# SimonRennotte/Data-Efficient-Reinforcement-Learning-with-Probabilistic-Model-Predictive-Control

Hardware: AMD Instinct MI355X
Metric: MPC trajectory rollouts/sec (higher is better)
Workload: dtype f64

## Files before the change

### data-efficient-reinforcement-learning-with-probabilistic-model-predictive-control_amd/_lib.py

```python
import ctypes as C
import os

_HERE = os.path.dirname(os.path.abspath(__file__))
LIB_PATH = os.environ.get("GPMPC_LIB") or os.path.join(_HERE, "libgpmpc_hip.so")

GPMPC_OK = 0
GPMPC_ERR_ARG = -1
GPMPC_ERR_NOT_PD = -2
GPMPC_ERR_HIP = -3
GPMPC_ERR_LIMIT = -4


class GpmpcError(RuntimeError):
    def __init__(self, code, msg):
        super().__init__(f"gpmpc error {code}: {msg}")
        self.code = code


class NotPositiveDefiniteError(GpmpcError):
    """Cholesky failure of K + noise*I -- the reference lets torch.linalg.cholesky's error
    propagate uncaught (rl_gp_mpc/control_objects/models/gp_model.py:427)."""


_P = C.c_void_p
_D = C.c_double
_I = C.c_int

SIGNATURES = {
    "gpmpc_abi_version": (C.c_int, []),
    "gpmpc_create": (C.c_int, [C.POINTER(_P), _I]),
    "gpmpc_destroy": (C.c_int, [_P]),
    "gpmpc_last_error": (C.c_char_p, [_P]),
    "gpmpc_prepare": (C.c_int, [_P, _P, _P, _P, _P, _P, _I, _I, _I, _P]),
    "gpmpc_prepare_sparse": (C.c_int, [_P, _P, _P, _I, _P, _I, _P, _P, _P, _D, _I, _I, _P]),
    "gpmpc_sparse_append": (C.c_int, [_P, _P, _P, _I, _I, _I, _P]),
    "gpmpc_sparse_forget": (C.c_int, [_P, _P, _P, _I, _I, _I, _P]),
    "gpmpc_select_inducing": (C.c_int, [_P, _P, _I, _I, _P, _P, _D, _I, _I, _P, _P, _P, _P]),
    "gpmpc_set_factors": (C.c_int, [_P, _P, _P, _P, _P, _P, _I, _I, _I, _P]),
    "gpmpc_get_factors": (C.c_int, [_P, C.POINTER(_P), C.POINTER(_P)]),
    "gpmpc_read_factors": (C.c_int, [_P, _P, _P, _P]),
    "gpmpc_predict": (C.c_int, [_P, _P, _I, _I, _I, _P, _P, _P, _P]),
    "gpmpc_predict_backward": (C.c_int, [_P, _P, _I, _I, _I, _P, _P, _P, _P]),
    "gpmpc_predict_cov": (C.c_int, [_P, _P, _I, _P, _I, _I, _I, _P, _P, _P]),
    "gpmpc_moments": (C.c_int, [_P, _P, _P, _I, _I, _I, _P, _P, _P, _P]),
    "gpmpc_moments_linear": (C.c_int, [_P, _P, _P, _I, _I, _I, _P, _P, _P, _P]),
    "gpmpc_moments_backward": (C.c_int, [_P, _P, _P, _I, _I, _I, _P, _P, _P, _P, _P, _P]),
    "gpmpc_moments_linear_backward": (C.c_int, [_P, _P, _P, _I, _I, _I, _P, _P, _P, _P, _P, _P]),
    "gpmpc_forget": (C.c_int, [_P, C.POINTER(_I), _I, _P]),
    "gpmpc_last_prepare_mode": (C.c_int, [_P]),
    "gpmpc_last_rollout_path": (C.c_int, [_P]),
    "gpmpc_last_grad_path": (C.c_int, [_P]),
    "gpmpc_last_cluster": (C.c_int, [_P]),
    "gpmpc_build_id": (C.c_char_p, []),
    "gpmpc_mll": (C.c_int, [_P, _P, _P, _P, _P, _P, _I, _I, _I, C.POINTER(_D), _P]),
    "gpmpc_set_option": (C.c_int, [_P, C.c_char_p, C.c_longlong]),
    "gpmpc_set_cost": (C.c_int, [_P, _P, _P, _P, _D, _I, _P, _P, _I, _I]),
    "gpmpc_rollout": (C.c_int, [_P, _P, _P, _P, _I, _I, _I, _I, _D, _P, _P, _P, _P, _P, _P]),
    "gpmpc_rollout_linear": (C.c_int, [_P, _P, _P, _P, _I, _I, _I, _I, _D, _P, _P, _P, _P, _P, _P]),
    "gpmpc_rollout_linear_feedback": (C.c_int, [_P, _P, _P, _I, _P, _P, _I, _I, _I, _I, _D, _P, _P, _P, _P, _P, _P]),
    "gpmpc_lqr_gains": (C.c_int, [_P, _P, _P, _I, _I, _I, _I, _D, _D, _P, _P, _P, _P]),
    "gpmpc_rollout_grad": (C.c_int, [_P, _P, _P, _P, _I, _I, _I, _I, _D, _P, _P, _P, _P, _P, _P, _P]),
    "gpmpc_rollout_backward": (C.c_int, [_P, _P, _P, _P, _I, _I, _I, _I, _D, _P, _P, _P, _P, _P, _P, _P, _P, _P]),
    "gpmpc_rollout_linear_backward": (C.c_int, [_P, _P, _P, _P, _I, _I, _I, _I, _D, _P, _P, _P, _P, _P, _P, _P, _P, _P]),
    "gpmpc_rollout_linear_feedback_backward": (C.c_int, [_P, _P, _P, _I, _P, _P, _I, _I, _I, _I, _D, _P, _P, _P, _P, _P, _P, _P, _P,
                                                         _P, _P]),
    "gpmpc_objective_grad_host": (C.c_int, [_P, _P, _P, _P, _I, _I, _I, _D, C.POINTER(C.POINTER(_D)), _P]),
    "gpmpc_rollout_timed": (C.c_int, [_P, _P, _P, _P, _I, _I, _I, _I, _D, _P, _I, C.POINTER(C.c_float), _P]),
    "gpmpc_cem_search": (C.c_int, [_P, _P, _P, _I, _I, _I, _I, _D, _I, _I, C.c_ulonglong, _P, _I, _P, _P, _P, _P, _P]),
    "gpmpc_cem_local": (C.c_int, [_P, _P, _P, _I, _I, _I, _I, _I, _I, _D, _I, _I, C.c_ulonglong, _P, _I, _P, _P, _P, _P, _P, _P]),
    "gpmpc_cem_merge": (C.c_int, [_P, _P, _I, _I, _I, _I, _P, _P]),
    "gpmpc_argmin_async": (C.c_int, [_P, _P, _I, C.c_longlong, _P, _I, _P, _P]),
    "gpmpc_argmin_export": (C.c_int, [_P, _P, _I, C.c_longlong, _P, _I, _P, _P, _P]),
    "gpmpc_argmin": (C.c_int, [_P, _P, _I, C.c_longlong, C.POINTER(_D), C.POINTER(C.c_longlong), _P]),
}


ABI_VERSION = 24


def load(path=LIB_PATH):
    if not os.path.exists(path):
        raise ImportError(
            f"{path} not found: the HIP extension is required (no CPU fallback). "
            "Build it with `python __graft_entry__.py` or `make -C <package>/csrc`.")
    lib = C.CDLL(path)
    for name, (res, args) in SIGNATURES.items():
        fn = getattr(lib, name)
        fn.restype = res
        fn.argtypes = args
    if lib.gpmpc_abi_version() != ABI_VERSION:
        raise ImportError(f"{path}: ABI version {lib.gpmpc_abi_version()} != expected {ABI_VERSION}; rebuild the HIP library")
    return lib


_lib = None


def lib():
    global _lib
    if _lib is None:
        _lib = load()
    return _lib
```

### data-efficient-reinforcement-learning-with-probabilistic-model-predictive-control_amd/csrc/abi.hip

```cpp
#include <cmath>
#include <cstring>
#include <new>
#include <dlfcn.h>

#include "gpmpc_internal.h"
#include "lqr_gains_plan.h"

namespace {
struct Roctx {
    int (*push)(const char*) = nullptr;
    int (*pop)() = nullptr;
    Roctx() {
        for (const char* lib : {"librocprofiler-sdk-roctx.so", "libroctx64.so"}) {
            void* hnd = dlopen(lib, RTLD_LAZY | RTLD_LOCAL);
            if (!hnd) continue;
            push = reinterpret_cast<int (*)(const char*)>(dlsym(hnd, "roctxRangePushA"));
            pop = reinterpret_cast<int (*)()>(dlsym(hnd, "roctxRangePop"));
            if (push && pop) return;
            push = nullptr; pop = nullptr;
        }
    }
};
struct Range {
    static const Roctx& api() { static Roctx r; return r; }
// ... 222 lines not shown
    GPMPC_HIP_CHECK(h, hipSetDevice(h->device));
    const size_t DN = (size_t)h->D * h->N;
    if (iK_dst) GPMPC_HIP_CHECK(h, hipMemcpyAsync(iK_dst, h->iK.p, DN * h->N * sizeof(double), hipMemcpyDeviceToDevice, (hipStream_t)stream));
    if (beta_dst) GPMPC_HIP_CHECK(h, hipMemcpyAsync(beta_dst, h->beta.p, DN * sizeof(double), hipMemcpyDeviceToDevice, (hipStream_t)stream));
    return GPMPC_OK;
}

int gpmpc_predict(gpmpc_t* g, const double* Xq, int M, int D, int E, const double* noises_host, double* mean_out,
                  double* var_out, void* stream) {
    Range roctx_range("gpmpc_predict");
    if (!g) return GPMPC_ERR_ARG;
    Handle* h = H_(g);
    if (!h->ready) return bad(g, "predict before prepare / set_factors / mll");
    if (D != h->D || E != h->E) return bad(g, "predict: D / E differ from the cached model");
    if (M < 0) return bad(g, "predict: M < 0");
    if (M > 0 && !Xq) return bad(g, "null argument");
    if (M == 0) return GPMPC_OK;
    GPMPC_HIP_CHECK(h, hipSetDevice(h->device));
    return run_predict(h, Xq, M, noises_host, mean_out, var_out, (hipStream_t)stream);
}

int gpmpc_predict_backward(gpmpc_t* g, const double* Xq, int M, int D, int E, const double* mean_bar, const double* var_bar,
                           double* Xq_bar_out, void* stream) {
    Range roctx_range("gpmpc_predict_backward");
    if (!g) return GPMPC_ERR_ARG;
    Handle* h = H_(g);
    if (!h->ready) return bad(g, "predict_backward before prepare / set_factors / mll");
    if (D != h->D || E != h->E) return bad(g, "predict_backward: D / E differ from the cached model");
    if (M < 0) return bad(g, "predict_backward: M < 0");
    if (M > 0 && (!Xq || !Xq_bar_out)) return bad(g, "null argument");
    if (M == 0) return GPMPC_OK;
    GPMPC_HIP_CHECK(h, hipSetDevice(h->device));
    return run_predict_backward(h, Xq, M, mean_bar, var_bar, Xq_bar_out, (hipStream_t)stream);
}

int gpmpc_predict_cov(gpmpc_t* g, const double* Xa, int Ma, const double* Xb, int Mb, int D, int E, const double* noises_host,
                      double* cov_out, void* stream) {
    Range roctx_range("gpmpc_predict_cov");
    if (!g) return GPMPC_ERR_ARG;
    Handle* h = H_(g);
    if (!h->ready) return bad(g, "predict_cov before prepare / set_factors / mll");
    if (D != h->D || E != h->E) return bad(g, "predict_cov: D / E differ from the cached model");
    if (Ma < 0 || (Xb && Mb < 0)) return bad(g, "predict_cov: negative number of points");
    if (Xb && noises_host) return bad(g, "predict_cov: the cross form takes no noise");
    if (Ma > (1 << 22) || (Xb && Mb > (1 << 22))) return bad(g, "predict_cov: more than 2^22 points");
    if (Ma == 0 || (Xb && Mb == 0)) return GPMPC_OK;
    if (!Xa || !cov_out) return bad(g, "null argument");
    GPMPC_HIP_CHECK(h, hipSetDevice(h->device));
    return run_predict_cov(h, Xa, Ma, Xb, Mb, noises_host, cov_out, (hipStream_t)stream);
}

int gpmpc_moments(gpmpc_t* g, const double* mu, const double* var, int P, int D, int E, double* M_out, double* S_out,
                  double* V_out, void* stream) {
    Range roctx_range("gpmpc_moments");
    if (!g) return GPMPC_ERR_ARG;
    Handle* h = H_(g);
    if (!h->ready) return bad(g, "moments before prepare / set_factors / mll");
    if (D > GPMPC_MAX_D || E > GPMPC_MAX_E) {
        h->err = "moments: D or E beyond the compiled limits";
        return GPMPC_ERR_LIMIT;
    }
    if (D != h->D || E != h->E) return bad(g, "moments: D / E differ from the cached model");
    if (P < 0) return bad(g, "moments: P < 0");
    if (P > 0 && (!mu || !M_out)) return bad(g, "null argument");
    if (P == 0) return GPMPC_OK;
    GPMPC_HIP_CHECK(h, hipSetDevice(h->device));
    return run_moments(h, mu, var, P, M_out, S_out, V_out, (hipStream_t)stream);
}

int gpmpc_moments_linear(gpmpc_t* g, const double* mu, const double* var, int P, int D, int E, double* M_out, double* S_out,
                         double* V_out, void* stream) {
    Range roctx_range("gpmpc_moments_linear");
    if (!g) return GPMPC_ERR_ARG;
    Handle* h = H_(g);
    if (!h->ready) return bad(g, "moments_linear before prepare / set_factors / mll");
    if (D > GPMPC_MAX_D || E > GPMPC_MAX_E) {
        h->err = "moments_linear: D or E beyond the compiled limits";
        return GPMPC_ERR_LIMIT;
    }
    if (D != h->D || E != h->E) return bad(g, "moments_linear: D / E differ from the cached model");
    if (P < 0) return bad(g, "moments_linear: P < 0");
    if (P > 0 && !mu) return bad(g, "null argument");
    if (P == 0) return GPMPC_OK;
    GPMPC_HIP_CHECK(h, hipSetDevice(h->device));
    return run_moments_linear(h, mu, var, P, M_out, S_out, V_out, (hipStream_t)stream);
}

int gpmpc_moments_backward(gpmpc_t* g, const double* mu, const double* var, int P, int D, int E, const double* M_bar,
                           const double* S_bar, const double* V_bar, double* mu_bar_out, double* var_bar_out, void* stream) {
    Range roctx_range("gpmpc_moments_backward");
    if (!g) return GPMPC_ERR_ARG;
    Handle* h = H_(g);
    if (!h->ready) return bad(g, "moments_backward before prepare / set_factors / mll");
    if (D > GPMPC_MAX_D || E > GPMPC_MAX_E) {
        h->err = "moments_backward: D or E beyond the compiled limits";
        return GPMPC_ERR_LIMIT;
    }
    if (D != h->D || E != h->E) return bad(g, "moments_backward: D / E differ from the cached model");
    if (P < 0) return bad(g, "moments_backward: P < 0");
    if (P > 0 && !mu) return bad(g, "null argument");
    if (P == 0) return GPMPC_OK;
    GPMPC_HIP_CHECK(h, hipSetDevice(h->device));
    return run_moments_backward(h, mu, var, P, M_bar, S_bar, V_bar, mu_bar_out, var_bar_out, (hipStream_t)stream);
}

int gpmpc_moments_linear_backward(gpmpc_t* g, const double* mu, const double* var, int P, int D, int E, const double* M_bar,
                                  const double* S_bar, const double* V_bar, double* mu_bar_out, double* var_bar_out,
                                  void* stream) {
    Range roctx_range("gpmpc_moments_linear_backward");
    if (!g) return GPMPC_ERR_ARG;
    Handle* h = H_(g);
    if (!h->ready) return bad(g, "moments_linear_backward before prepare / set_factors / mll");
    if (D > GPMPC_MAX_D || E > GPMPC_MAX_E) {
        h->err = "moments_linear_backward: D or E beyond the compiled limits";
        return GPMPC_ERR_LIMIT;
    }
    if (D != h->D || E != h->E) return bad(g, "moments_linear_backward: D / E differ from the cached model");
    if (P < 0) return bad(g, "moments_linear_backward: P < 0");
    if (P > 0 && !mu) return bad(g, "null argument");
    if (P == 0) return GPMPC_OK;
    GPMPC_HIP_CHECK(h, hipSetDevice(h->device));
    return run_moments_linear_backward(h, mu, var, P, M_bar, S_bar, V_bar, mu_bar_out, var_bar_out, (hipStream_t)stream);
}

int gpmpc_mll(gpmpc_t* g, const double* X, const double* Y, const double* ls, const double* os, const double* noise,
              int N, int D, int E, double* out_host, void* stream) {
    Range roctx_range("gpmpc_mll");
    if (!g) return GPMPC_ERR_ARG;
    if (!X || !Y || !ls || !os || !noise || !out_host) return bad(g, "null argument");
    int rc = check_dims(g, N, D, E);
    if (rc) return rc;
    GPMPC_HIP_CHECK(H_(g), hipSetDevice(g->h.device));
    return run_mll(H_(g), X, Y, ls, os, noise, N, D, E, out_host, (hipStream_t)stream);
}

int gpmpc_forget(gpmpc_t* g, const int* idx_host, int k, void* stream) {
    Range roctx_range("gpmpc_forget");
    if (!g) return GPMPC_ERR_ARG;
    Handle* h = H_(g);
    if (!h->ready || !h->have_state) return bad(g, "forget: the handle holds no record of a gpmpc_prepare");
    if (!idx_host) return bad(g, "null argument");
    if (k < 1 || k >= h->N) return bad(g, "forget: need 1 <= k < N");
    for (int q = 0; q < k; ++q)
        if (idx_host[q] < 0 || idx_host[q] >= h->N || (q > 0 && idx_host[q] <= idx_host[q - 1]))
            return bad(g, "forget: indices must be strictly ascending and in [0, N)");
    GPMPC_HIP_CHECK(h, hipSetDevice(h->device));
    return run_forget(h, idx_host, k, (hipStream_t)stream);
}

int gpmpc_last_prepare_mode(gpmpc_t* g) { return g ? g->h.last_prepare_mode : GPMPC_ERR_ARG; }

int gpmpc_last_rollout_path(gpmpc_t* g) { return g ? g->h.last_rollout_path : GPMPC_ERR_ARG; }
int gpmpc_last_cluster(gpmpc_t* g) { return g ? g->h.last_cluster : GPMPC_ERR_ARG; }

int gpmpc_last_grad_path(gpmpc_t* g) { return g ? g->h.last_grad_path : GPMPC_ERR_ARG; }

#ifndef GPMPC_BUILD_ID
#define GPMPC_BUILD_ID "unknown"
#endif
const char* gpmpc_build_id(void) { return GPMPC_BUILD_ID; }

int gpmpc_set_cost(gpmpc_t* g, const double* target, const double* W, const double* W_T, double kappa,
                   int clip, const double* smin, const double* smax, int D, int A) {
    if (!g || !target || !W || !W_T) return bad(g, "null argument");
    if (D < 1 || A < 0 || D > kMaxD || D + A > kMaxE) return bad(g, "bad D / A");
    if ((smin == nullptr) != (smax == nullptr)) return bad(g, "state_min and state_max must both be given or both be NULL");
    Handle* h = H_(g);
    GPMPC_HIP_CHECK(h, hipSetDevice(h->device));
    const int DA = D + A;
    const size_t n = (size_t)DA + (size_t)DA * DA + (size_t)D * D + 2 * (size_t)D;
    int rc = grow(h, h->cost, n);
    if (rc) return rc;
    double host[kMaxE + kMaxE * kMaxE + kMaxD * kMaxD + 2 * kMaxD];
    double* q = host;
    memcpy(q, target, DA * sizeof(double)); q += DA;
    memcpy(q, W, (size_t)DA * DA * sizeof(double)); q += DA * DA;
    memcpy(q, W_T, (size_t)D * D * sizeof(double)); q += D * D;
    for (int d = 0; d < D; ++d) q[d] = smin ? smin[d] : 0.0;
    q += D;
    for (int d = 0; d < D; ++d) q[d] = smax ? smax[d] : 0.0;
    GPMPC_HIP_CHECK(h, hipMemcpy(h->cost.p, host, n * sizeof(double), hipMemcpyHostToDevice));
    h->cost_D = D; h->cost_A = A; h->kappa = kappa; h->clip = clip; h->use_constraints = smin ? 1 : 0;
    return GPMPC_OK;
}

static int fill_args(gpmpc_t* g, RolloutArgs& a, const double* actions, const double* mu0, const double* S0,
                     int B, int H, int A, int include_time, double time0, bool need_cost = true) {
    Handle* h = H_(g);
    if (!h->ready) return bad(g, "rollout before prepare / set_factors");
    if (!actions || !mu0 || !S0) return bad(g, "null argument");
    if (B < 1 || H < 1 || A < 0) return bad(g, "need B >= 1, H >= 1");
    if (h->D + A + (include_time ? 1 : 0) != h->E) return bad(g, "D + A (+1 with time) must equal the model's input dim E");
    if (need_cost && (h->cost_D != h->D || h->cost_A != A)) return bad(g, "gpmpc_set_cost not called for this (D, A)");
    memset(&a, 0, sizeof a);
    a.Xt = h->Xt.p; a.beta = h->beta.p; a.Tm = h->Tm.p; a.ils2 = h->ils2.p; a.var = h->var.p; a.logvar = h->logvar.p;
    a.cost = h->cost.p; a.kappa = h->kappa; a.clip = h->clip; a.use_constraints = h->use_constraints;
    a.actions = actions;
    a.N = h->N; a.D = h->D; a.A = A; a.E = h->E; a.H = H; a.B = B;
    a.include_time = include_time; a.time0 = time0;
    memcpy(a.mu0, mu0, h->D * sizeof(double));
    memcpy(a.S0, S0, (size_t)h->D * h->D * sizeof(double));
    return GPMPC_OK;
}

int gpmpc_rollout(gpmpc_t* g, const double* actions, const double* mu0, const double* S0, int B, int H, int A,
                  int include_time, double time0, double* mu_out, double* Sig_out, double* cm_out, double* cv_out,
                  double* J_out, void* stream) {
    Range roctx_range("gpmpc_rollout");
    if (!g) return GPMPC_ERR_ARG;
    RolloutArgs a;
    int rc = fill_args(g, a, actions, mu0, S0, B, H, A, include_time, time0, cm_out || cv_out || J_out);
    if (rc) return rc;
    GPMPC_HIP_CHECK(H_(g), hipSetDevice(g->h.device));
    a.mu_out = mu_out; a.Sig_out = Sig_out; a.cm_out = cm_out; a.cv_out = cv_out; a.J_out = J_out;
    return launch_rollout(H_(g), a, (hipStream_t)stream);
}

int gpmpc_rollout_linear(gpmpc_t* g, const double* actions, const double* mu0, const double* S0, int B, int H, int A,
                         int include_time, double time0, double* mu_out, double* Sig_out, double* cm_out, double* cv_out,
                         double* J_out, void* stream) {
    Range roctx_range("gpmpc_rollout_linear");
    if (!g) return GPMPC_ERR_ARG;
    RolloutArgs a;
    int rc = fill_args(g, a, actions, mu0, S0, B, H, A, include_time, time0, cm_out || cv_out || J_out);
    if (rc) return rc;
    GPMPC_HIP_CHECK(H_(g), hipSetDevice(g->h.device));
    a.mu_out = mu_out; a.Sig_out = Sig_out; a.cm_out = cm_out; a.cv_out = cv_out; a.J_out = J_out;
    return run_rollout_linear(H_(g), a, (hipStream_t)stream);
}

int gpmpc_rollout_linear_feedback(gpmpc_t* g, const double* actions, const double* gains, int gains_per_candidate,
                                  const double* mu0, const double* S0, int B, int H, int A, int include_time, double time0,
                                  double* mu_out, double* Sig_out, double* cm_out, double* cv_out, double* J_out, void* stream) {
    if (!gains)
        return gpmpc_rollout_linear(g, actions, mu0, S0, B, H, A, include_time, time0, mu_out, Sig_out, cm_out, cv_out, J_out,
                                    stream);
    Range roctx_range("gpmpc_rollout_linear_feedback");
    if (!g) return GPMPC_ERR_ARG;
    RolloutArgs a;
    int rc = fill_args(g, a, actions, mu0, S0, B, H, A, include_time, time0, cm_out || cv_out || J_out);
    if (rc) return rc;
    if (A < 1) return bad(g, "feedback gains need A >= 1");
    GPMPC_HIP_CHECK(H_(g), hipSetDevice(g->h.device));
    a.mu_out = mu_out; a.Sig_out = Sig_out; a.cm_out = cm_out; a.cv_out = cv_out; a.J_out = J_out;
    return run_rollout_linear(H_(g), a, (hipStream_t)stream, gains, gains_per_candidate != 0);
}

int gpmpc_lqr_gains(gpmpc_t* g, const double* actions, const double* mu0, int B, int H, int A, int include_time, double time0,
                    double reg, double* gains_out, double* P_out, int* flags_out, void* stream) {
    Range roctx_range("gpmpc_lqr_gains");
    if (!g) return GPMPC_ERR_ARG;
    Handle* h = H_(g);
    if (!h->ready) return bad(g, "lqr_gains before prepare / set_factors");
    if (!actions || !mu0 || !gains_out) return bad(g, "null argument");
    if (B < 1 || H < 1 || A < 1) return bad(g, "lqr_gains: need B >= 1, H >= 1, A >= 1");
    if (h->D + A + (include_time ? 1 : 0) != h->E) return bad(g, "D + A (+1 with time) must equal the model's input dim E");
    if (!(reg >= 0.0) || !std::isfinite(reg)) return bad(g, "lqr_gains: reg must be finite and >= 0");
    if (A > kLqrMaxA) {
        h->err = "lqr_gains: A beyond the compiled limit (A <= 8)";
        return GPMPC_ERR_LIMIT;
    }
    if (h->cost_D != h->D || h->cost_A != A) return bad(g, "gpmpc_set_cost not called for this (D, A)");
    GPMPC_HIP_CHECK(h, hipSetDevice(h->device));
    return run_lqr_gains(h, actions, mu0, B, H, A, include_time, time0, reg, gains_out, P_out, flags_out, (hipStream_t)stream);
}

int gpmpc_rollout_grad(gpmpc_t* g, const double* actions, const double* mu0, const double* S0, int B, int H, int A,
                       int include_time, double time0, double* J_out, double* grad_out, double* mu_out, double* Sig_out,
                       double* cm_out, double* cv_out, void* stream) {
    Range roctx_range("gpmpc_rollout_grad");
    if (!g) return GPMPC_ERR_ARG;
    if (!grad_out) return bad(g, "null argument");
    RolloutArgs a;
    int rc = fill_args(g, a, actions, mu0, S0, B, H, A, include_time, time0);
    if (rc) return rc;
    if (A < 1) return bad(g, "gradient needs A >= 1");
    GPMPC_HIP_CHECK(H_(g), hipSetDevice(g->h.device));
    a.mu_out = mu_out; a.Sig_out = Sig_out; a.J_out = J_out; a.cm_out = cm_out; a.cv_out = cv_out;
    return launch_rollout_grad(H_(g), a, grad_out, (hipStream_t)stream);
}

int gpmpc_rollout_backward(gpmpc_t* g, const double* actions, const double* mu0, const double* S0, int B, int H, int A,
                           int include_time, double time0, const double* mu_bar, const double* Sig_bar, const double* cm_bar,
                           const double* cv_bar, const double* J_bar, double* actions_bar_out, double* mu0_bar_out,
                           double* S0_bar_out, void* stream) {
    Range roctx_range("gpmpc_rollout_backward");
    if (!g) return GPMPC_ERR_ARG;
    if (!actions_bar_out) return bad(g, "null argument");
    RolloutSeeds sd{mu_bar, Sig_bar, cm_bar, cv_bar, J_bar, mu0_bar_out, S0_bar_out, cm_bar || cv_bar || J_bar};
    RolloutArgs a;
    int rc = fill_args(g, a, actions, mu0, S0, B, H, A, include_time, time0, sd.cost);
    if (rc) return rc;
    if (A < 1) return bad(g, "gradient needs A >= 1");
    GPMPC_HIP_CHECK(H_(g), hipSetDevice(g->h.device));
    return launch_rollout_grad(H_(g), a, actions_bar_out, (hipStream_t)stream, &sd);
}

int gpmpc_rollout_linear_backward(gpmpc_t* g, const double* actions, const double* mu0, const double* S0, int B, int H, int A,
                                  int include_time, double time0, const double* mu_bar, const double* Sig_bar,
                                  const double* cm_bar, const double* cv_bar, const double* J_bar, double* actions_bar_out,
                                  double* mu0_bar_out, double* S0_bar_out, void* stream) {
    Range roctx_range("gpmpc_rollout_linear_backward");
    if (!g) return GPMPC_ERR_ARG;
    if (!actions_bar_out) return bad(g, "null argument");
    RolloutSeeds sd{mu_bar, Sig_bar, cm_bar, cv_bar, J_bar, mu0_bar_out, S0_bar_out, cm_bar || cv_bar || J_bar};
    RolloutArgs a;
// ... 260 lines not shown
```

### data-efficient-reinforcement-learning-with-probabilistic-model-predictive-control_amd/csrc/gpmpc_internal.h

```cpp
#pragma once
#include <hip/hip_runtime.h>
#include <cstddef>
#include <cstdio>
#include <string>
#include <unordered_set>

#include "../../include/gpmpc.h"

namespace gpmpc_hip {

constexpr int kMaxD = GPMPC_MAX_D;
constexpr int kMaxE = GPMPC_MAX_E;
constexpr int kWave = 64;

struct ClusterMap {
    int CS, D, P, P_off, wpp, wtri, koff;
    int CSd;
    unsigned char sepown[8];
    unsigned char meanown[4];
    unsigned char dmem[32];
    unsigned char didx[32];
    __host__ __device__ int diag_owner(int ord, int slot) const { return dmem[((ord * wtri + slot) * CSd) / (D * wtri)]; }
    __host__ __device__ int off_owner(int ord, int slot) const { return ((slot * koff) / wpp + ord * koff) % CS; }
    __host__ __device__ int sep_owner(int ord) const { return sepown[ord]; }
// ... 33 lines not shown
                for (int k = 1; k < koff; ++k) {
                    const int m = (o * koff + k) % CS;
                    if (diag_count(m) <= diag_count(best)) best = m;
                }
            sepown[o] = (unsigned char)best;
            taken[best] = true;
        }
        if (dedicated) {
            CSd = 0;
            for (int m = 0; m < 32; ++m) didx[m] = 255;
            for (int m = 0; m < CS; ++m)
                if (!taken[m]) { dmem[CSd] = (unsigned char)m; didx[m] = (unsigned char)CSd; ++CSd; }
        }
        for (int a = 0; a < D && a < 4; ++a) {
            int pick = -1;
            for (int m = CS - 1, k = 0; m >= 0 && pick < 0; --m)
                if (!taken[m]) { if (k == a) pick = m; ++k; }
            meanown[a] = (unsigned char)(pick >= 0 ? pick : (a * CS / D) % CS);
        }
    }
};

constexpr int kInlineActs = 64;
struct RolloutArgs {
    const double* Xt;
    const double* beta;
    const double* Tm;
    const double* ils2;
    const double* var;
    const double* logvar;
    const double* cost;
    double kappa;
    int clip;
    int use_constraints;
    const double* actions;
    int N, D, A, E, H, B;
    int B_plan;
    int include_time;
    double time0;
    double* mu_out;
    double* Sig_out;
    double* cm_out;
    double* cv_out;
    double* J_out;
    const double* xrange;
    const int* mono_exp;
    const double* mono_w;
    int mono_cum[16];
    int sep_kmax;
    int CM;
    int force_path;
    int force_sep;
    int x_in_lds;
    int cols2;
    int G;
    int CH;
    int RC;
    unsigned magic_N;
    unsigned magic_wpp;
    unsigned magic_pt;
    int tiled;
    int t_begin, t_end;
    int ntiles;
    const double* tile_part;
    const int* slow;
    double* grad_mom;
    int* grad_done;
    int grad_NSP, grad_NXP;
    int cluster;
    ClusterMap cmap;
    int cl_slots;
    int xch_n;
    unsigned xch_tag0;
    unsigned long long* xch;
    unsigned long long* xch_uc;
    int cl_dbg;
    int act_inline_n;
    double* act_store;
    double act_inline[kInlineActs];
    double mu0[kMaxD];
    double S0[kMaxD * kMaxD];
};

struct Buf {
    double* p = nullptr;
    size_t cap = 0;
};

struct Handle {
    int device = 0;
    std::string err;
    int N = 0, D = 0, E = 0;
    bool ready = false;
    Buf Xt;
    Buf beta;
    Buf iK;
    Buf Tm;
    Buf ils2;
    Buf var;
    Buf logvar;
    Buf gram;
    Buf linv;
    Buf zvec;
    Buf cost;
    Buf best;
    Buf traj;
    Buf xrange;
    Buf gradws;
    Buf mllws;
    Buf cemws;
    Buf tilews;
    Buf tgradws;
    Buf predws;
    Buf predbws;
    Buf covws;
    Buf momws;
    Buf mombws;
    Buf linws;
    Buf linbws;
    Buf lqrws;
    struct SepTable* septab = nullptr;
    Buf sepw;
    int septab_D = -1, sep_ks = 0, sep_cmax = 0;
    hipStream_t side_stream = nullptr;
    hipEvent_t ev_params = nullptr, ev_points = nullptr;
    Buf Xc, Yc;
    Buf hyp;
    Buf kv, vv;
    Buf sc;
    int* mismatch = nullptr;
    int inc_updates = 0;
    bool have_state = false;
    Buf Xf, Yf;
    Buf fgws;
    Buf spws;
    Buf selws;
    int* fidx = nullptr;
    size_t fidx_cap = 0;
    Buf hio;
    double* hio_host = nullptr;
    double* hio_host_dev = nullptr;
    size_t hio_host_cap = 0;
    unsigned long long* hio_flag = nullptr;
    unsigned long long* hio_flag_dev = nullptr;
    unsigned long long hio_seq = 0;
    double* hx_out = nullptr; const double* hx_src = nullptr; int hx_n = 0;
    Buf xch;
    unsigned long long* xch_uc = nullptr;
    size_t xch_uc_cap = 0;
    unsigned xch_epoch = 1;
    int opt_cluster = 0;
    int opt_cl_dbg = 0;
    int last_cluster = 1;
    Buf mono_w;
    int* mono_exp = nullptr;
    int mono_D = -1;
    int mono_cum[16] = {0};
    int sep_kmax = 0;
    int mono_CM = 0;
    int* info = nullptr;
    std::unordered_set<const void*> lds_configured;
    int cost_D = -1, cost_A = -1;
    double kappa = 1.0;
    int clip = 0;
    int use_constraints = 0;
    int opt_threads = 0;
    int opt_lds_kb = 0;
    int opt_force_global = 0;
    int opt_rows_per_chunk = 0;
    int opt_force_path = 0;
    int opt_force_sep = 0;
    int opt_grad_stream = 0;
    int opt_grad_share = 0;
    int opt_grad_chunk = 0;
    int chunk_key[8] = {0, 0, 0, 0, 0, 0, 0, 0};
    int chunk_rows = 0;
    int opt_grad_tiles = 1;
    int opt_grad_sep = 1;
    int opt_cols_per_lane = 0;
    int opt_incremental = 1;
    int opt_refresh_every = 32;
    int opt_outer2 = 2;
    int opt_outer_min_n = 640;
    int opt_block128 = 1;
    int opt_inner_left = 1;
    int opt_tile128 = 1;
    int opt_outer_block = 1;
    int opt_pair_tiles = 0;
    int last_rollout_path = 0;
    int opt_grad_mean = 1;
    int last_grad_path = 0;
    int opt_prepare_inv_batch = 4;
    int opt_prepare_invcols = 1;
    int opt_prepare_fuse = 1;
    int opt_prepare_overlap = 1;
    int opt_gram_shared = 1;
    int opt_fused_prepare = 1;
    int last_prepare_mode = 0;
    int opt_sparse_chunk = 0;
    long long opt_select_max_mb = 0;
    int opt_predict_chunk = 0;
    int opt_predict_bwd_chunk = 0;
    int opt_predict_cov_chunk = 0;
    int opt_moments_chunk = 0;
    int opt_moments_bwd_chunk = 0;
    int opt_moments_linear_chunk = 0;
    int opt_moments_linear_bwd_chunk = 0;
    int opt_lqr_gains_chunk = 0;
    int lds_limit = 160 * 1024;
    int num_cu = 256;
    Buf sprec;
    bool sp_have = false;
    size_t sp_yu = 0;
    Buf spupd;
};

inline int allow_full_lds(Handle* h, const void* kernel);

#define GPMPC_HIP_CHECK(h, expr)                                                         \
    do {                                                                                 \
        hipError_t e_ = (expr);                                                          \
        if (e_ != hipSuccess) {                                                          \
            (h)->err = std::string(#expr) + ": " + hipGetErrorString(e_);                \
            return GPMPC_ERR_HIP;                                                        \
        }                                                                                \
    } while (0)

inline int allow_full_lds(Handle* h, const void* kernel) {
    if (h->lds_configured.count(kernel)) return GPMPC_OK;
    GPMPC_HIP_CHECK(h, hipFuncSetAttribute(kernel, hipFuncAttributeMaxDynamicSharedMemorySize, h->lds_limit));
    h->lds_configured.insert(kernel);
    return GPMPC_OK;
}

inline unsigned magic_div(unsigned d) { return d <= 1 ? 0u : (unsigned)((0x100000000ULL + d - 1) / d); }

constexpr double kTileTableBytes = 6.0e6;
inline bool tables_outgrow_l2(int N, int D) { return 4.0 * D * (double)N * N >= kTileTableBytes; }

struct RolloutRequest {
    bool fused_tiles;
    bool costs_to_caller;
};
struct RolloutPlan {
    int DP;
    int nt;
    int path;
    int cols2, G, CH, RC, x_in_lds;
    size_t lds_bytes;
    int cluster, cl_slots, xch_n;
    ClusterMap cmap;
    unsigned magic_N, magic_wpp, magic_pt;
    int CM, sep_kmax;
    bool fused_tiles;
    bool costs_to_caller;
    const char* err;
};

struct MomTiling {
    int G, CH, RC, wpp, gz;
    size_t lds;
};
struct GradPlan {
    int DP, NXP, RS, NSP;
    int sweep_nt, pre_steps;
    size_t sweep_lds;
    bool stream;
    size_t gs_lds;
    MomTiling first;
    MomTiling pass;
    bool share_cu;
    bool tiles, fused;
    bool sep;
    int sep_kmax, sep_NA, sep_NE, sep_PS, sep_wave_words;
    size_t sep_lds;
    int pairs_left;
    bool few, merged;
    int path;
    RolloutPlan fwd;
};

constexpr int kSmallPathMaxN = 240;
constexpr int kSmallCholeskyMinN = 96;
constexpr int kInvColsMaxN = 352;
constexpr int kInvColsWideMaxN = 544;
constexpr int kSyrkTiledMinN = 512;
constexpr int kGramSharedTilesPerCu = 2;

enum class PreparePath {
    small_whole,
    small_cholesky,
    panel32,
    outer,
};
enum class GramForm { full, lower, shared_lower };
enum class Inv32Form { rows, cols, side };
enum class OuterInvForm { rows128, doubling, doubling_ykk };
enum class SyrkInvForm { w32, tiled, t128 };
struct PreparePlan {
    PreparePath path;
    GramForm gram;
    bool round2;
    bool fuse_next;
    Inv32Form inv32;
    int inv_batch;
    bool tile128;
// ... 101 lines not shown
```

### data-efficient-reinforcement-learning-with-probabilistic-model-predictive-control_amd/csrc/rollout.hip

```cpp
#include "rollout_stream_kernel.h"

namespace gpmpc_hip {

int launch_rollout_dp2(Handle*, RolloutArgs&, int, bool, size_t, hipStream_t);
int launch_rollout_dp3(Handle*, RolloutArgs&, int, bool, size_t, hipStream_t);
int launch_rollout_dp4(Handle*, RolloutArgs&, int, bool, size_t, hipStream_t);
int launch_rollout_dp6(Handle*, RolloutArgs&, int, bool, size_t, hipStream_t);
int launch_rollout_dp8(Handle*, RolloutArgs&, int, bool, size_t, hipStream_t);
int launch_rollout_dp16(Handle*, RolloutArgs&, int, bool, size_t, hipStream_t);

__global__ __launch_bounds__(64) void traj_cost_kernel(const double* __restrict__ mu, const double* __restrict__ Sig,
                                                       const double* __restrict__ actions, const double* __restrict__ cost,
                                                       int D, int A, int H, double kappa, int clip, int use_constraints,
                                                       double* __restrict__ cm_out, double* __restrict__ cv_out,
                                                       double* __restrict__ J_out) {
    traj_cost_body(blockIdx.x, threadIdx.x, mu, Sig, actions, cost, D, A, H, kappa, clip, use_constraints, cm_out, cv_out, J_out);
}

__device__ __forceinline__ void keep_better(double& bv, long long& bi, double ov, long long oi) {
    if (oi >= 0 && (bi < 0 || ov < bv || (ov == bv && oi < bi))) { bv = ov; bi = oi; }
}

__global__ __launch_bounds__(1024) void argmin_kernel(const double* J, int B, long long first, double* out, int index_as_double,
                                                     const double* actions, int HA, double* out_host) {
// ... 231 lines not shown
        const int items = D * wtri, P_off = D * (D - 1) / 2;
        const int cs_floor = (P_off + 2 * D > 9) ? P_off + 2 * D : 9;
        const bool roomy = cap >= cs_floor;
        int cs = 1;
        if (h.opt_cluster >= 2) cs = h.opt_cluster;
        else if (items >= 24 || (roomy && items * D >= 18)) {
            cs = (items + 3) / 4;
            if (roomy && cs < cs_floor) cs = cs_floor;
        }
        if (cs > 32) cs = 32;
        if (cs > cap) cs = cap;
        for (const int cs_min = h.opt_cluster >= 2 ? cs : (cs + 1) / 2; cs >= 2 && cs >= cs_min && cluster == 1; --cs) {
            p.cmap.plan(cs, D, wpp_c, wtri);
            p.cl_slots = 0;
            for (int m = 0; m < cs; ++m) { const int n = p.cmap.slots_needed(m); if (n > p.cl_slots) p.cl_slots = n; }
            for (int xl = ((size_t)E * N * 8 <= 32 * 1024) ? 1 : 0; xl >= 0 && cluster == 1; --xl) {
                const Layout L = make_layout(N, D, A, E, P, DP, wpp_c, CM, CH, H * A, xl != 0, true, p.cl_slots);
                if ((size_t)L.lds_total * 8 <= lds_cap) { G = P; lds_bytes = (size_t)L.lds_total * 8; p.x_in_lds = xl; cluster = cs; }
            }
        }
        if (cluster > 1 && h.opt_threads == 0) nt = cluster >= 8 ? 512 : 1024;
        if (cluster == 1) cl_chunks = false;
    }
    if (!gs && cluster == 1) {
        choose_layout(false);
        if (G == 0) { gs = true; tiled = false; }
    }
    if (gs) {
        if (DP % 4 == 0 && DP >= 8) {
            CH = (N >= 1024) ? 256 : 64;
            if (h.opt_rows_per_chunk > 0) CH = h.opt_rows_per_chunk <= 64 ? 64 : (h.opt_rows_per_chunk <= 128 ? 128 : 256);
        } else {
            CH = (N >= 64) ? 64 : ((N + 3) & ~3);
        }
        RC = (N + CH - 1) / CH;
        G = 1;
        StreamLayout SL = make_stream_layout(N, D, A, E, DP, CH, H * A);
        lds_bytes = (size_t)SL.total * 8;
        if (lds_bytes > (size_t)h.lds_limit) { p.err = "rollout: N too large for the LDS column-factor array"; return GPMPC_ERR_LIMIT; }
        nt = 1024;
    }
    p.cols2 = (cols2 && !gs) ? 1 : 0;
    const int NCf = p.cols2 ? NCu : N;
    const unsigned wppv = (unsigned)((RC * NCf + 63) / 64);
    p.magic_N = magic_div((unsigned)NCf);
    p.magic_wpp = magic_div(wppv);
    p.magic_pt = magic_div((unsigned)N);
    if ((unsigned long long)RC * NCf * NCf >= 0x100000000ULL || (unsigned long long)G * wppv * wppv >= 0x100000000ULL ||
        (!gs && (unsigned long long)(D + 2 * P) * N * N >= 0x100000000ULL)) {
        p.err = "rollout: index range too large for the multiply-high division"; return GPMPC_ERR_LIMIT;
    }
    if (!gs && (unsigned long long)G * wppv >= 65000ULL) {
        p.err = "rollout: too many work-item slots for the 16-bit item list"; return GPMPC_ERR_LIMIT;
    }
    p.nt = nt; p.path = gs ? 1 : (tiled ? 2 : 0);
    p.G = G; p.CH = CH; p.RC = RC; p.lds_bytes = lds_bytes;
    p.cluster = cluster;
    if (cluster > 1) p.xch_n = G * (int)wppv + G + D * (D + 1) + 32;
    p.fused_tiles = tiled && req.fused_tiles;
    p.costs_to_caller = req.costs_to_caller;
    return GPMPC_OK;
}

static int exchange_buffers(Handle* h, RolloutArgs& a, const RolloutPlan& p, hipStream_t s) {
    const size_t words = (size_t)8 * ((a.B + 7) / 8) * 4 * p.xch_n;
    const bool fresh = !h->xch.p || words > h->xch.cap;
    int rc = grow(h, h->xch, words);
    if (rc) return rc;
    const bool wrap = h->xch_epoch >= (1u << 19) - 1;
    if (fresh || wrap) { rc = zero_exchange(h, reinterpret_cast<unsigned long long*>(h->xch.p), h->xch.cap, s); if (rc) return rc; }
    if (words > h->xch_uc_cap) {
        if (h->xch_uc) GPMPC_HIP_CHECK(h, hipFree(h->xch_uc));
        h->xch_uc = nullptr; h->xch_uc_cap = 0;
        void* q = nullptr;
        if (hipExtMallocWithFlags(&q, words * sizeof(unsigned long long), hipDeviceMallocUncached) != hipSuccess) {
            (void)hipGetLastError();
            GPMPC_HIP_CHECK(h, hipExtMallocWithFlags(&q, words * sizeof(unsigned long long), hipDeviceMallocFinegrained));
        }
        h->xch_uc = reinterpret_cast<unsigned long long*>(q);
        h->xch_uc_cap = words;
        rc = zero_exchange(h, h->xch_uc, words, s);
        if (rc) return rc;
    } else if (wrap) {
        rc = zero_exchange(h, h->xch_uc, h->xch_uc_cap, s);
        if (rc) return rc;
    }
    if (wrap) h->xch_epoch = 1;
    a.xch_tag0 = h->xch_epoch * 8192u;
    h->xch_epoch += 1;
    a.xch = reinterpret_cast<unsigned long long*>(h->xch.p);
    a.xch_uc = h->xch_uc;
    return GPMPC_OK;
}

int launch_rollout(Handle* h, RolloutArgs& a, const RolloutPlan& p, hipStream_t s) {
    const bool tiled = p.path == 2;
    a.xrange = h->xrange.p; a.mono_exp = h->mono_exp; a.mono_w = h->mono_w.p;
    for (int k = 0; k < 16; ++k) a.mono_cum[k] = h->mono_cum[k];
    a.sep_kmax = p.sep_kmax; a.CM = p.CM;
    a.force_path = h->opt_force_path; a.force_sep = h->opt_force_sep;
    a.x_in_lds = p.x_in_lds; a.cols2 = p.cols2;
    a.G = p.G; a.CH = p.CH; a.RC = p.RC;
    a.magic_N = p.magic_N; a.magic_wpp = p.magic_wpp; a.magic_pt = p.magic_pt;
    a.cluster = p.cluster; a.cmap = p.cmap; a.cl_slots = p.cl_slots; a.cl_dbg = h->opt_cl_dbg;
    a.xch = nullptr; a.xch_uc = nullptr; a.xch_n = p.xch_n; a.xch_tag0 = 0;
    a.tiled = tiled ? 1 : 0;
    if (!p.fused_tiles) a.grad_mom = nullptr;
    if (!tiled) { a.t_begin = 0; a.t_end = 0; a.slow = nullptr; a.tile_part = nullptr; a.ntiles = 0; }
    if (a.act_inline_n > 0 && p.path != 0) {
        InlineActs u;
        for (int i = 0; i < kInlineActs; ++i) u.v[i] = a.act_inline[i];
        hipLaunchKernelGGL(inline_acts_kernel, dim3(1), dim3(64), 0, s, a.act_store, a.act_inline_n, u);
        GPMPC_HIP_CHECK(h, hipGetLastError());
        a.act_inline_n = 0;
    }
    if (!a.mu_out || !a.Sig_out) {
        const size_t nmu = (size_t)a.B * (a.H + 1) * a.D, nS = nmu * a.D;
        int rc = grow(h, h->traj, nmu + nS);
        if (rc) return rc;
        if (!a.mu_out) a.mu_out = h->traj.p;
        if (!a.Sig_out) a.Sig_out = h->traj.p + nmu;
    }
    int rc = p.cluster > 1 ? exchange_buffers(h, a, p, s) : GPMPC_OK;
    if (rc) return rc;
    auto launch_kernel = [&]() {
        const bool gs = p.path == 1;
        switch (p.DP) {
            case 2:  return launch_rollout_dp2(h, a, p.nt, gs, p.lds_bytes, s);
            case 3:  return launch_rollout_dp3(h, a, p.nt, gs, p.lds_bytes, s);
            case 4:  return launch_rollout_dp4(h, a, p.nt, gs, p.lds_bytes, s);
            case 6:  return launch_rollout_dp6(h, a, p.nt, gs, p.lds_bytes, s);
            case 8:  return launch_rollout_dp8(h, a, p.nt, gs, p.lds_bytes, s);
            default: return launch_rollout_dp16(h, a, p.nt, gs, p.lds_bytes, s);
        }
    };
    if (tiled) {
        rc = tile_workspace(h, a);
        if (!rc) rc = launch_tile_state_init(h, a, s);
        for (int t = 0; t < a.H && !rc; ++t) {
            rc = launch_pair_tiles(h, a, t, s);
            a.t_begin = t; a.t_end = t + 1;
            if (!rc) rc = launch_kernel();
        }
    } else {
        rc = launch_kernel();
    }
    if (rc) return rc;
    if ((a.cm_out || a.cv_out || a.J_out) && !p.costs_to_caller) {
        rc = launch_traj_cost(h, a, a.cm_out, a.cv_out, a.J_out, s);
        if (rc) return rc;
    }
    h->last_rollout_path = p.path;
    h->last_cluster = p.cluster;
    return GPMPC_OK;
}

int launch_rollout(Handle* h, RolloutArgs& a, hipStream_t s) {
    int rc = ensure_rollout_tables(h, a.N, a.D);
    if (rc) return rc;
    RolloutPlan p;
    rc = plan_rollout(*h, a.N, a.D, a.A, a.E, a.H, a.B_plan > a.B ? a.B_plan : a.B, RolloutRequest{false, false}, p);
    if (rc) { h->err = p.err; return rc; }
    return launch_rollout(h, a, p, s);
}

}
```

### data-efficient-reinforcement-learning-with-probabilistic-model-predictive-control_amd/csrc/rollout_kernel.h

```cpp
#pragma once
#include "device_common.h"

#if defined(GPMPC_PROF_ON)
#define GPMPC_TRACE(id) do { if (threadIdx.x == 0 && blockIdx.x == 0) { long long now_ = __builtin_readcyclecounter(); \
    prof_acc[id] += now_ - prof_last; prof_last = now_; } \
    if (CL && threadIdx.x == 0 && (blockIdx.x & 7) == 0) { long long w_ = wall_clock64(); prof_wall[id] += w_ - prof_wlast; prof_wlast = w_; } } while (0)
#else
#define GPMPC_TRACE(id) do {} while (0)
#endif

namespace gpmpc_hip {

typedef const __attribute__((address_space(3))) double* lds_cptr;
__device__ inline double lds_b64(const double* p) {
    lds_cptr q = (lds_cptr)p;
    asm volatile("" : "+v"(q));
    return *q;
}

typedef double lds_d2 __attribute__((ext_vector_type(2)));
template <int NL, int NV>
__device__ inline void lds_load_pairs(const double* rec, double (&v)[NV]) {
    static_assert(NV >= ((NL + 1) & ~1), "destination too short");
    const lds_d2* r2 = reinterpret_cast<const lds_d2*>(rec);
// ... 435 lines not shown
#pragma unroll
        for (int u = 0; u < U; ++u) {
            double r[RS];
            REC::template load<RS>(rec + u * RS, r);
            double x = r[REC::EA] + kb0, y = r[REC::EA] + kb1;
#pragma unroll
            for (int d = 0; d < DP; ++d) { x = fma(r[REC::G + d], w0[d], x); y = fma(r[REC::G + d], w1[d], y); }
            a0[u] = x; a1[u] = y;
            if (diag) t_row_pair(t, so + (unsigned)u * t.row_bytes, wt0[u], wt1[u]);
            else { wt0[u] = r[REC::RA]; wt1[u] = r[REC::RA]; }
        }
#pragma unroll
        for (int u = 0; u < U; ++u) {
            acc0 = fma(fast_exp(a0[u], tab), wt0[u], acc0);
            acc1 = fma(fast_exp(a1[u], tab), wt1[u], acc1);
        }
        rec += U * RS;
        so += (unsigned)U * t.row_bytes;
    }
}

__device__ inline double wave_sum8(const double (&v)[8], int lane) {
    auto xchg = [](double x, int mask) { return __shfl_xor(x, mask, 64); };
    const bool b0 = lane & 1, b1 = lane & 2, b2 = lane & 4;
    double r4[4], r2[2];
#pragma unroll
    for (int k = 0; k < 4; ++k) {
        const double keep = b0 ? v[k + 4] : v[k], send = b0 ? v[k] : v[k + 4];
        r4[k] = keep + xchg(send, 1);
    }
#pragma unroll
    for (int k = 0; k < 2; ++k) {
        const double keep = b1 ? r4[k + 2] : r4[k], send = b1 ? r4[k] : r4[k + 2];
        r2[k] = keep + xchg(send, 2);
    }
    double r = (b2 ? r2[1] : r2[0]) + xchg(b2 ? r2[0] : r2[1], 4);
    r += xchg(r, 8);
    r += xchg(r, 16);
    r += xchg(r, 32);
    return r;
}

constexpr int sep3_bands(int KS) { return KS <= 3 ? 2 : (KS == 4 ? 3 : (KS == 5 ? 5 : 7)); }
constexpr int sep3_i0(int B, int KS) {
    if (KS <= 4) return B;
    if (KS == 5) return B < 2 ? 0 : B - 1;
    return B < 2 ? 0 : (B < 4 ? 1 : B - 2);
}
constexpr int sep3_i1(int B, int KS) { return B == sep3_bands(KS) - 1 ? KS : sep3_i0(B, KS); }
constexpr int sep3_j0(int B, int KS) {
    if (KS == 5) return B == 1 ? 2 : 0;
    if (KS >= 6) return (B == 1 || B == 3) ? 2 : 0;
    return 0;
}
constexpr int sep3_j1(int B, int KS) {
    if (KS == 5) return B == 0 ? 1 : KS;
    if (KS >= 6) return (B == 0 || B == 2) ? 1 : KS;
    return KS;
}
constexpr int sep3_count(int B, int KS) {
    int n = 0;
    if (B >= sep3_bands(KS)) return 0;
    for (int i = sep3_i0(B, KS); i <= sep3_i1(B, KS) && i <= KS; ++i)
        for (int j = sep3_j0(B, KS); j <= sep3_j1(B, KS) && j <= KS - i; ++j) n += KS - i - j + 1;
    return n;
}
template <int KS, int B>
struct Sep3Canon {
    int v[sep3_count(B, KS) > 0 ? sep3_count(B, KS) : 1];
    constexpr Sep3Canon() : v{} {
        int n = 0;
        for (int i = sep3_i0(B, KS); i <= sep3_i1(B, KS) && i <= KS && B < sep3_bands(KS); ++i)
            for (int j = sep3_j0(B, KS); j <= sep3_j1(B, KS) && j <= KS - i; ++j)
                for (int kk = 0; kk <= KS - i - j; ++kk) {
                    const int deg = i + j + kk;
                    const int cum = deg * (deg + 1) * (deg + 2) / 6;
                    v[n++] = cum + (deg - i) * (deg - i + 1) / 2 + (deg - i - j);
                }
    }
};

template <int KS, int B>
__device__ inline void sep3_band(int lane, int N, int side, const double* rec0, int RS, const double* kb, const double* nu,
                                 const double* il, double* mom) {
    constexpr int NBm = sep3_count(B, KS);
    if constexpr (NBm > 0) {
        constexpr int NP = (NBm + 7) & ~7;
        constexpr int I0 = sep3_i0(B, KS), I1 = sep3_i1(B, KS) < KS ? sep3_i1(B, KS) : KS;
        constexpr int J0 = sep3_j0(B, KS), J1 = sep3_j1(B, KS);
        double acc[NP];
#pragma unroll
        for (int m = 0; m < NP; ++m) acc[m] = 0.0;
        for (int pt = lane; pt < N; pt += 64) {
            double x0, x1, x2, wt;
            if (side == 0) {
                double r[RowRecAligned<3>::RS];
                RowRecAligned<3>::load<RowRecAligned<3>::RS>(rec0 + (size_t)pt * RS, r);
                wt = r[RowRecAligned<3>::RA]; x0 = r[0]; x1 = r[1]; x2 = r[2];
            } else {
                wt = kb[pt];
                x0 = nu[pt] * il[0]; x1 = nu[N + pt] * il[1]; x2 = nu[2 * N + pt] * il[2];
            }
            double py[KS + 1], pz[KS + 1];
            py[0] = 1.0; pz[0] = 1.0;
#pragma unroll
            for (int e = 1; e <= KS; ++e) { py[e] = py[e - 1] * x1; pz[e] = pz[e - 1] * x2; }
            double wx = wt;
#pragma unroll
            for (int e = 0; e < I0; ++e) wx *= x0;
            int n = 0;
#pragma unroll
            for (int i = I0; i <= I1; ++i) {
#pragma unroll
                for (int j = J0; j <= (J1 < KS - i ? J1 : KS - i); ++j) {
                    const double aij = wx * py[j];
#pragma unroll
                    for (int kk = 0; kk <= KS - i - j; ++kk) { acc[n] = fma(aij, pz[kk], acc[n]); ++n; }
                }
                wx *= x0;
            }
        }
        static constexpr Sep3Canon<KS, B> canon{};
        const int mq = lane >> 2;
#pragma unroll
        for (int g16 = 0; g16 + 16 <= NP; g16 += 16) {
            const double(&grp)[16] = *reinterpret_cast<const double(*)[16]>(&acc[g16]);
            const double tot = wave_reduce16(grp);
            if ((lane & 3) == 0 && g16 + mq < NBm) mom[canon.v[g16 + mq]] = tot;
        }
        if constexpr (NP % 16 != 0) {
            constexpr int g8 = NP - 8;
            const double(&grp)[8] = *reinterpret_cast<const double(*)[8]>(&acc[g8]);
            const double tot = wave_reduce8(grp);
            if ((lane & 3) == 0 && lane < 32 && g8 + mq < NBm) mom[canon.v[g8 + mq]] = tot;
        }
    }
}

template <int KS>
__device__ __attribute__((noinline)) void sep3_item(int band, int lane, int N, int side, const double* rec0, int RS,
                                                     const double* kb, const double* nu, const double* il, double* mom) {
    switch (band) {
        case 0: sep3_band<KS, 0>(lane, N, side, rec0, RS, kb, nu, il, mom); break;
        case 1: sep3_band<KS, 1>(lane, N, side, rec0, RS, kb, nu, il, mom); break;
        case 2: sep3_band<KS, 2>(lane, N, side, rec0, RS, kb, nu, il, mom); break;
        case 3: sep3_band<KS, 3>(lane, N, side, rec0, RS, kb, nu, il, mom); break;
        case 4: sep3_band<KS, 4>(lane, N, side, rec0, RS, kb, nu, il, mom); break;
        case 5: sep3_band<KS, 5>(lane, N, side, rec0, RS, kb, nu, il, mom); break;
        default: sep3_band<KS, 6>(lane, N, side, rec0, RS, kb, nu, il, mom); break;
    }
}

template <int DP, bool CL>
constexpr int rollout_min_waves() { return (DP == 2 || (DP == 3 && !CL)) ? 4 : 1; }

template <int DP, int NT, int DX, bool C2, bool TILED = false, bool CL = false>
__global__ __launch_bounds__(NT, (rollout_min_waves<DP, CL>())) void rollout_kernel(const RolloutArgs p) {
    static_assert(!TILED || (DP <= 4 && NT >= 256), "the batch-major path is built for D <= 4");
    static_assert(!CL || (!TILED && DP <= 4 && NT >= 256), "the cooperative form is built for D <= 4");
    extern __shared__ __attribute__((aligned(16))) double smem[];
    if constexpr (TILED) {
        if (p.slow[blockIdx.x] != p.t_begin + 1) return;
    }
    constexpr int NW = NT / kWave;
    using REC = RowRecAligned<DP>;
    constexpr int RS = REC::RS;
    const int tid = threadIdx.x;
    const int CS = CL ? p.cluster : 1;
    const bool spread = CL && (p.cl_dbg & 8);
    const int member = CL ? (spread ? (int)blockIdx.x % CS : (int)(blockIdx.x >> 3) % CS) : 0;
    const int c = CL ? (spread ? (int)blockIdx.x / CS : (int)(blockIdx.x & 7) + 8 * ((int)(blockIdx.x >> 3) / CS)) : (int)blockIdx.x;
    if constexpr (CL) { if (c >= p.B) return; }
    const int D = (DX > 0) ? DX : p.D;
    const int N = p.N, A = p.A, E = p.E, H = p.H, G = p.G, CM = p.CM;
    const int P = TILED ? D * (D - 1) / 2 : D * (D + 1) / 2;
    const int DA = D + A;
    const int LD = 2 * D;
    const int NC = C2 ? (N + 1) / 2 : N;
    const int wpp = (p.RC * NC + 63) / 64;
    const int SD2 = rnd2(D * D);

    const Layout L = make_layout(N, D, A, E, G, DP, wpp, CM, p.CH, H * A, p.x_in_lds != 0, CL, CL ? p.cl_slots : 0);
    const int NR = N + p.CH;
    double* s_mu = smem + L.mu;
    double* s_Sig2 = smem + L.Sig;
    double* s_m = smem + L.m;
    double* s_M = smem + L.M;
    double* s_cc = smem + L.cc;
    double* s_s1 = smem + L.s1;
    double* s_Vs = smem + L.Vs;
    double* s_Sp = smem + L.Sp;
    double* s_rdet = smem + L.rdet;
    [[maybe_unused]] double* s_rdiag = smem + L.misc;
    double* s_aug = smem + L.aug;
    double* s_part = smem + L.part;
    double* s_mom = smem + L.mom;
    int* s_pa = reinterpret_cast<int*>(smem + L.ints);
    int* s_pb = s_pa + P;
    int* s_K = s_pb + P;
    int* s_counter = s_K + G;
    int* s_noff = s_counter + 1;
    int* s_off = s_noff + 1;
    int* s_mcum = s_off + G;
    int* s_tri = s_mcum + 16;
    int* s_nslot = s_tri + tri_ints(N);
    int* s_nitems = s_nslot + G;
    unsigned short* s_items = reinterpret_cast<unsigned short*>(
        smem + L.ints + rnd2((2 * P + 3 * G + 8 + 16 + tri_ints(N) + 1) / 2));

    [[maybe_unused]] double* s_sepv = smem + L.cl;
    [[maybe_unused]] int* s_ord = reinterpret_cast<int*>(smem + L.cl + rnd2(G));
    [[maybe_unused]] int* s_fail = reinterpret_cast<int*>(smem + L.cl + rnd2(G) + rnd2((G + 1) / 2));
    [[maybe_unused]] unsigned char* s_needw = reinterpret_cast<unsigned char*>(smem + L.cl + rnd2(G) + rnd2((G + 1) / 2) + 2);
    [[maybe_unused]] unsigned char* s_own = s_needw + kClusterScratch * 8;
    [[maybe_unused]] unsigned char* s_sepown = s_own + G * wpp;
    [[maybe_unused]] unsigned char* s_elneed = s_sepown + G;
    [[maybe_unused]] unsigned char* s_meanown = s_elneed + G;
    [[maybe_unused]] unsigned short* s_mine = reinterpret_cast<unsigned short*>(
        smem + L.cl + rnd2(G) + rnd2((G + 1) / 2) + 2 + kClusterScratch + rnd2((G * wpp + 2 * G + 16 + 7) / 8));
    [[maybe_unused]] int* s_slot = reinterpret_cast<int*>(smem + L.cl + rnd2(G) + rnd2((G + 1) / 2) + 2 + kClusterScratch +
                                                          rnd2((G * wpp + 2 * G + 16 + 7) / 8) + rnd2((G * wpp + 16 + 4 + 3) / 4));
    [[maybe_unused]] unsigned long long* s_mymask = reinterpret_cast<unsigned long long*>(
        smem + L.cl + rnd2(G) + rnd2((G + 1) / 2) + 2 + kClusterScratch + rnd2((G * wpp + 2 * G + 16 + 7) / 8) +
        rnd2((G * wpp + 16 + 4 + 3) / 4) + rnd2((G + 1) / 2));
    const int GL = CL ? p.cl_slots : G;

    [[maybe_unused]] unsigned long long* xbuf_uc = CL ? p.xch_uc + (size_t)c * 4 * p.xch_n : nullptr;
    [[maybe_unused]] unsigned long long* xbuf = CL ? p.xch + (size_t)c * 4 * p.xch_n : nullptr;
    [[maybe_unused]] const int x_sep = G * wpp, x_mean = G * wpp + G;
    [[maybe_unused]] const int x_xcc = x_mean + D * (D + 1);
    [[maybe_unused]] int* s_lmap = reinterpret_cast<int*>(smem + L.lmap);
    constexpr int LMS = CL ? kLaneMapSlotsCluster : kLaneMapSlots;
    [[maybe_unused]] int* s_lrows = s_lmap + (wpp < LMS ? wpp : LMS) * 64;
    double* ppbase = smem;
    double* a_nu = ppbase + L.nu;
    double* a_lb = ppbase + L.lb;
    double* a_rows = ppbase + L.rows;
    double* a_kb = ppbase + L.kb;

    double* c_ils2 = smem + L.c_ils2;
    double* c_logvar = smem + L.c_logvar;
    double* c_var = smem + L.c_var;
    double* c_xr = smem + L.c_xr;
    double* c_act = smem + L.c_act;
    double* c_exptab = smem + L.c_exptab;
    const double* Xs = p.x_in_lds ? (smem + L.c_X) : p.Xt;
    double* c_monow = smem + L.c_monow;
    int* c_monoe = reinterpret_cast<int*>(smem + L.c_monoe);
    const double* act = p.actions + (size_t)c * H * A;

#if defined(GPMPC_PROF_ON)
    long long prof_x[3] = {0, 0, 0};
    long long prof_acc[10] = {0, 0, 0, 0, 0, 0, 0, 0, 0, 0};
    long long prof_last = __builtin_readcyclecounter();
    long long prof_wall[10] = {0, 0, 0, 0, 0, 0, 0, 0, 0, 0};
    long long prof_wlast = wall_clock64();
#endif
    if constexpr (TILED) {
        for (int i = tid; i < D; i += NT) { s_mu[i] = p.mu_out[((size_t)c * (H + 1) + p.t_begin) * D + i]; c_logvar[i] = p.logvar[i]; c_var[i] = p.var[i]; }
        for (int i = tid; i < D * D; i += NT) s_Sig2[i] = p.Sig_out[((size_t)c * (H + 1) + p.t_begin) * D * D + i];
    }
    {
        const bool inl = p.act_inline_n > 0;
        const int CMc = CM > 0 ? CM : 0;
        const double* mw = CMc > 0 ? p.mono_w : p.ils2;
        const int* me = CMc > 0 ? p.mono_exp : reinterpret_cast<const int*>(p.ils2);
        const int im = tid < CMc ? tid : 0;
        const int nX = p.x_in_lds ? E * N : 0;
        __builtin_amdgcn_sched_barrier(0);
        const double v_lv = p.logvar[tid < D ? tid : 0], v_var = p.var[tid < D ? tid : 0];
        const double v_ils = p.ils2[tid < D * E ? tid : 0], v_xr = p.xrange[tid < 2 * E ? tid : 0];
        const double v_act = act[tid < H * A ? tid : 0];
        const double v_exp = kExp2Tab[tid & 63];
        const double v_mw = mw[im];
        const int e0 = me[im * 4], e1 = me[im * 4 + 1], e2 = me[im * 4 + 2], e3 = me[im * 4 + 3];
        const double v_x0 = p.Xt[tid < nX ? tid : 0], v_x1 = p.Xt[tid + NT < nX ? tid + NT : 0];
        [[maybe_unused]] const double v_mu0 = p.mu0[tid < D ? tid : 0], v_S0 = p.S0[tid < D * D ? tid : 0];
        __builtin_amdgcn_sched_barrier(0);
        if constexpr (!TILED) {
            if (tid < D) s_mu[tid] = v_mu0;
            if (tid < D * D) s_Sig2[tid] = v_S0;
        }
        if (tid < D) { c_logvar[tid] = v_lv; c_var[tid] = v_var; }
        if (tid < D * E) c_ils2[tid] = v_ils;
        if (tid < 2 * E) c_xr[tid] = v_xr;
        if (tid < 64) c_exptab[tid] = v_exp;
        if (tid < CMc) { c_monow[tid] = v_mw; c_monoe[tid] = e0 | (e1 << 8) | (e2 << 16) | (e3 << 24); }
        if (tid < nX) smem[L.c_X + tid] = v_x0;
        if (tid + NT < nX) smem[L.c_X + tid + NT] = v_x1;
        if (inl) {
            for (int i = tid; i < H * A; i += NT) {
                const double v = p.act_inline[i < kInlineActs ? i : 0];
                c_act[i] = v;
                if (!CL || member == 0) p.act_store[i] = v;
            }
        } else {
            if (tid < H * A) c_act[tid] = v_act;
            for (int i = tid + NT; i < H * A; i += NT) c_act[i] = act[i];
        }
        for (int i = tid + NT; i < D; i += NT) { c_logvar[i] = p.logvar[i]; c_var[i] = p.var[i]; }
        for (int i = tid + NT; i < D * E; i += NT) c_ils2[i] = p.ils2[i];
        for (int i = tid + NT; i < 2 * E; i += NT) c_xr[i] = p.xrange[i];
        for (int i = tid + 2 * NT; i < nX; i += NT) smem[L.c_X + i] = p.Xt[i];
        for (int i = tid + NT; i < CMc; i += NT) {
            c_monow[i] = p.mono_w[i];
            c_monoe[i] = p.mono_exp[i * 4] | (p.mono_exp[i * 4 + 1] << 8) | (p.mono_exp[i * 4 + 2] << 16) | (p.mono_exp[i * 4 + 3] << 24);
        }
    }
    for (int i = tid; i < GL * p.CH * RS; i += NT) {
        const int gq = i / (p.CH * RS), k = i - gq * (p.CH * RS);
        a_rows[((size_t)gq * NR + N) * RS + k] = 0.0;
    }
    if (tid >= 64 && tid < 80) s_mcum[tid - 64] = p.mono_cum[tid - 64];
    if (tid == 0) {
        int q = 0;
        [[maybe_unused]] int nd_ = 0, no_ = 0;
        for (int a = 0; a < D; ++a)
            for (int b = TILED ? a + 1 : a; b < D; ++b) {
                s_pa[q] = a; s_pb[q] = b;
                if constexpr (CL) s_ord[q] = (a == b) ? nd_++ : no_++;
                ++q;
            }
        if constexpr (CL) *s_fail = 0;
        int run = 0;
        for (int r = 0; r <= p.RC; ++r) {
            s_tri[r] = run;
            const int first = C2 ? (r * p.CH) / 2 : r * p.CH;
            run += (first < NC) ? NC - first : 0;
        }
    }
    __syncthreads();
    bool use_lmap = false;
    if constexpr (!TILED) {
        const int wtri = (s_tri[p.RC] + 63) >> 6;
        use_lmap = wtri <= LMS && wtri <= wpp;
        if (use_lmap) {
            for (int slot = tid >> 6; slot < wtri; slot += NW) {
                const int flat = slot * 64 + (tid & 63);
                const bool valid = flat < s_tri[p.RC];
                int lo = 0, hi = p.RC;
                while (hi - lo > 1) {
                    const int mid = (lo + hi) >> 1;
                    if (s_tri[mid] <= flat) lo = mid; else hi = mid;
                }
                const int r = valid ? lo : 0;
                const int first = C2 ? (r * p.CH) / 2 : r * p.CH;
                const int jc = valid ? first + (flat - s_tri[r]) : 0;
                const int j = C2 ? 2 * jc : jc;
                const int jl = (C2 && (j + 1 < N)) ? j + 1 : j;
                const int i0 = r * p.CH;
                int i1 = i0 + p.CH;
                if (i1 > N) i1 = N;
                if (i1 > jl + 1) i1 = jl + 1;
                const int len = (valid && i1 > i0) ? (i1 - i0) : 0;
                const int nrows = (wave_max_i32(len) + 3) & ~3;
                s_lmap[flat] = valid ? (r | (jc << 8)) : -1;
                if ((tid & 63) == 0) s_lrows[slot] = nrows;
            }
        }
        __syncthreads();
    }
    GPMPC_TRACE(1);
    if (!TILED && member == 0) {
        for (int i = tid; i < D; i += NT) p.mu_out[((size_t)c * (H + 1)) * D + i] = s_mu[i];
        for (int i = tid; i < D * D; i += NT) p.Sig_out[((size_t)c * (H + 1)) * D * D + i] = s_Sig2[i];
    }

    [[maybe_unused]] const int wtri_c = CL ? (s_tri[p.RC] + 63) >> 6 : 0;
    if constexpr (CL) {
        const ClusterMap& cmap = p.cmap;
        for (int i = tid; i < P * wpp; i += NT) {
            const int gq = i / wpp, slot = i - gq * wpp, ord = s_ord[gq];
            int o;
            if (s_pa[gq] == s_pb[gq]) o = slot < wtri_c ? cmap.diag_owner(ord, slot) : 255;
            else o = cmap.off_owner(ord, slot);
            s_own[i] = (unsigned char)o;
        }
        for (int gq = tid; gq < P; gq += NT) {
            const int ord = s_ord[gq];
            const bool dg = s_pa[gq] == s_pb[gq];
            s_sepown[gq] = (unsigned char)(dg ? 255 : cmap.sep_owner(ord));
            s_elneed[gq] = (dg ? cmap.diag_needed(ord, member) : cmap.off_needed(ord, member)) ? 1 : 0;
        }
        for (int a = tid; a < D; a += NT) s_meanown[a] = (unsigned char)cmap.mean_owner(a);
        __syncthreads();
        if (tid == 0) {
            int n = 0;
            for (int gq = 0; gq < P; ++gq) s_slot[gq] = s_elneed[gq] ? n++ : -1;
            if (n > GL) *s_fail = 1;
        }
        for (int gq = tid >> 6; gq < P; gq += NT / 64) {
            const int k = tid & 63;
            const int lim = (s_pa[gq] == s_pb[gq]) ? wtri_c : wpp;
            const unsigned long long m = __ballot(k < lim && k < wpp && s_own[gq * wpp + (k < wpp ? k : 0)] == member);
            if (k == 0) s_mymask[gq] = m;
        }
        __syncthreads();
    }
    [[maybe_unused]] auto item_owner = [&](int code) -> int {
        if (code >= 0xffff - 15) return s_meanown[0xffff - code];
        const int gq = p.magic_wpp ? (int)__umulhi((unsigned)code, p.magic_wpp) : code;
        return (s_K[gq] & 64) ? s_sepown[gq] : s_own[code];
    };
    [[maybe_unused]] auto pair_needed = [&](int gq) -> bool { return (s_K[gq] & 64) ? s_sepown[gq] == member : s_elneed[gq] != 0; };
    [[maybe_unused]] unsigned x_tag = 0;
    [[maybe_unused]] unsigned long long* x_cur = xbuf;
    [[maybe_unused]] bool same_xcd = false;
    [[maybe_unused]] auto publish = [&](int vi, double v) {
        unsigned long long* g = x_cur + 2 * (size_t)vi;
        const unsigned long long hi_tag = (unsigned long long)x_tag << 32;
        if (same_xcd) {
            __hip_atomic_store(g, hi_tag | (unsigned)__double2loint(v), __ATOMIC_RELAXED, __HIP_MEMORY_SCOPE_WORKGROUP);
            __hip_atomic_store(g + 1, hi_tag | (unsigned)__double2hiint(v), __ATOMIC_RELAXED, __HIP_MEMORY_SCOPE_WORKGROUP);
        } else {
            __hip_atomic_store(g, hi_tag | (unsigned)__double2loint(v), __ATOMIC_RELAXED, __HIP_MEMORY_SCOPE_AGENT);
            __hip_atomic_store(g + 1, hi_tag | (unsigned)__double2hiint(v), __ATOMIC_RELAXED, __HIP_MEMORY_SCOPE_AGENT);
        }
    };
    [[maybe_unused]] auto acquire = [&](int vi) -> double {
        const unsigned long long* g = x_cur + 2 * (size_t)vi;
        for (int spins = 0; spins < (1 << 21); ++spins) {
            const unsigned long long a = __hip_atomic_load(g, __ATOMIC_RELAXED, __HIP_MEMORY_SCOPE_AGENT);
            const unsigned long long b = __hip_atomic_load(g + 1, __ATOMIC_RELAXED, __HIP_MEMORY_SCOPE_AGENT);
            if ((unsigned)(a >> 32) == x_tag && (unsigned)(b >> 32) == x_tag) return __hiloint2double((int)(unsigned)b, (int)(unsigned)a);
            __builtin_amdgcn_s_sleep(1);
        }
        *s_fail = 1;
        return __builtin_nan("");
    };

    if constexpr (CL) {
        x_tag = p.xch_tag0;
        x_cur = xbuf + (size_t)2 * p.xch_n;
        const int my_xcc = __builtin_amdgcn_s_getreg(20 | (0 << 6) | ((4 - 1) << 11));
        if (tid == 0) publish(x_xcc + member, (double)my_xcc);
        if (tid < 64) {
            const bool differs = tid < CS && acquire(x_xcc + tid) != (double)my_xcc;
            const unsigned long long any_differs = __ballot(differs);
            if (tid == 0) s_fail[1] = (any_differs == 0 && !(p.cl_dbg & 4)) ? 1 : 0;
        }
        __syncthreads();
        same_xcd = s_fail[1] != 0;
        if (*s_fail) {
            if (member == 0) {
                for (int i = tid; i < H * D; i += NT) p.mu_out[((size_t)c * (H + 1) + 1) * D + i] = __builtin_nan("");
                for (int i = tid; i < H * D * D; i += NT) p.Sig_out[((size_t)c * (H + 1) + 1) * D * D + i] = __builtin_nan("");
            }
            return;
        }
    }

    int cur = 0;
    const int tid_outer = tid;
    for (int t = TILED ? p.t_begin : 0; t < (TILED ? p.t_end : H); ++t) {
        int tid_opaque = tid_outer;
        asm volatile("" : "+v"(tid_opaque));
        const int tid = tid_opaque;
        const int lane = tid & 63;
        const int wave = tid >> 6;
        const double* s_Sig = s_Sig2 + cur * SD2;
        double* s_SigNext = s_Sig2 + (cur ^ 1) * SD2;
        if constexpr (CL) {
            x_tag = p.xch_tag0 + (unsigned)t + 1u;
            x_cur = (same_xcd ? xbuf : xbuf_uc) + (size_t)(t & 1) * 2 * p.xch_n;
        }

        for (int q0 = 0; q0 < P || (TILED && q0 == 0); q0 += G) {
            const int Gc = (P - q0 < G) ? (P - q0) : G;
            const bool first = (q0 == 0);
            const int nmean = first ? D : 0;

            constexpr int kPairBase = (NT >= 256) ? 64 : 0;
#if defined(GPMPC_PROF_ON)
            const long long prof_p1 = __builtin_readcyclecounter();
#endif
            if (first) {
                for (int i = tid; i < E; i += NT) {
                    double v;
                    if (i < D) v = s_mu[i];
                    else if (i < DA) v = c_act[t * A + (i - D)];
                    else v = p.time0 + (double)t;
                    s_m[i] = v;
                }
            }
            if (tid < nmean) {
                const int a = tid;
                double* aug = s_aug + a * (D * LD);
                double prodil = 1.0;
                double detA;
                if constexpr (DP <= 4) {
                    double m[DP][2 * DP];
#pragma unroll
                    for (int i = 0; i < DP; ++i) {
                        const double il2 = (i < D) ? c_ils2[a * E + i] : 1.0;
                        prodil *= il2;
#pragma unroll
                        for (int j = 0; j < DP; ++j) {
                            const bool in = (i < D && j < D);
                            m[i][j] = (in ? s_Sig[i * D + j] : 0.0) + (i == j ? 1.0 / il2 : 0.0);
                            m[i][DP + j] = (in && i == j) ? 1.0 : 0.0;
                        }
                    }
                    detA = small_solve<DP>(m);
#pragma unroll
                    for (int i = 0; i < DP; ++i)
#pragma unroll
                        for (int j = 0; j < DP; ++j)
                            if (i < D && j < D) aug[i * LD + D + j] = m[i][DP + j];
                } else {
                    for (int i = 0; i < D; ++i) {
                        const double il2 = c_ils2[a * E + i];
                        prodil *= il2;
                        for (int j = 0; j < D; ++j) {
                            aug[i * LD + j] = s_Sig[i * D + j] + (i == j ? 1.0 / il2 : 0.0);
                            aug[i * LD + D + j] = (i == j ? 1.0 : 0.0);
                        }
                    }
                    detA = gauss_solve(aug, D, D, LD);
                }
                s_cc[a] = c_var[a] / sqrt(detA * prodil);
            } else if (tid >= kPairBase + (kPairBase ? 0 : nmean) && tid < kPairBase + (kPairBase ? 0 : nmean) + Gc) {
                const int gq = tid - kPairBase - (kPairBase ? 0 : nmean);
                const int a = s_pa[q0 + gq], b = s_pb[q0 + gq];
                double* aug = s_aug + (D + gq) * (D * LD);
                double detR;
                double cmax = 0.0;
                if constexpr (DP <= 4) {
                    double m[DP][2 * DP];
#pragma unroll
                    for (int i = 0; i < DP; ++i)
#pragma unroll
                        for (int j = 0; j < DP; ++j) {
                            const bool in = (i < D && j < D);
                            const double sg = in ? s_Sig[i * D + j] : 0.0;
                            const double dab = in ? c_ils2[a * E + j] + c_ils2[b * E + j] : 0.0;
                            m[i][j] = sg * dab + (i == j ? 1.0 : 0.0);
                            m[i][DP + j] = sg;
                        }
                    double ur[DP], wr[DP];
#pragma unroll
                    for (int i = 0; i < DP; ++i) {
                        const double mi = (i < D) ? s_mu[i] : 0.0;
                        const double rg = (i < D) ? fmax(fabs(c_xr[i] - mi), fabs(c_xr[E + i] - mi)) : 0.0;
                        ur[i] = (i < D) ? rg * c_ils2[a * E + i] : 0.0;
                        wr[i] = (i < D) ? rg * c_ils2[b * E + i] : 0.0;
                    }
                    detR = small_solve<DP>(m);
                    double rowc[DP];
#pragma unroll
                    for (int i = 0; i < DP; ++i) {
                        double r = 0.0;
#pragma unroll
                        for (int j = 0; j < DP; ++j) {
                            if (i < D && j < D) {
                                aug[i * LD + D + j] = m[i][DP + j];
                                r = fma(fabs(m[i][DP + j]), wr[j], r);
                            }
                        }
                        rowc[i] = r * ur[i];
                    }
#pragma unroll
                    for (int i = 0; i < DP; ++i) cmax += rowc[i];
                } else {
                    for (int i = 0; i < D; ++i)
                        for (int j = 0; j < D; ++j) {
                            const double dab = c_ils2[a * E + j] + c_ils2[b * E + j];
                            aug[i * LD + j] = s_Sig[i * D + j] * dab + (i == j ? 1.0 : 0.0);
                            aug[i * LD + D + j] = s_Sig[i * D + j];
                        }
                    detR = gauss_solve(aug, D, D, LD);
                    const double* Z = aug + D;
                    for (int i = 0; i < D; ++i) {
                        const double mi = s_mu[i];
                        const double ui = fmax(fabs(c_xr[i] - mi), fabs(c_xr[E + i] - mi)) * c_ils2[a * E + i];
                        for (int j = 0; j < D; ++j) {
                            const double mj = s_mu[j];
                            const double wj = fmax(fabs(c_xr[j] - mj), fabs(c_xr[E + j] - mj)) * c_ils2[b * E + j];
                            cmax = fma(fabs(Z[i * LD + j]) * ui, wj, cmax);
                        }
                    }
                }
                s_rdet[gq] = 1.0 / sqrt(detR);
                int K = 0;
                if (p.force_path != 1 && cmax <= kTaylorMaxArg[kMaxTaylor]) {
                    K = 1;
#pragma unroll
                    for (int k = 1; k < kMaxTaylor; ++k) K += (cmax > kTaylorMaxArg[k]) ? 1 : 0;
                }
                if (a != b && K > 0 && K <= p.sep_kmax && (DX != 3 || K <= 6) && p.force_path == 0) {
                    const long long C_ = s_mcum[K < 3 ? 3 : K];
                    const long long NBk = (s_mcum[K] + 7) / 8;
                    const long long cost_sep = (DX == 3) ? 2 * (((N + 63) / 64) * (2 * C_ + 40) + (C_ / 8 + 4) * 70)
                                                         : 2 * NBk * (((N + 63) / 64) * (6 + 8 * K) + 80);
                    const long long cost_el = (long long)N * N * (D + K + 3) / 64;
                    if (p.force_sep || cost_sep < cost_el) K |= 64;
                }
                if constexpr (CL) K |= (s_slot[gq] + 1) << 8;
                s_K[gq] = K;
            }
            if constexpr (TILED) {
                if (first && tid >= 128 && tid < 128 + D) {
                    const int a = tid - 128;
                    double m[DP][2 * DP];
#pragma unroll
                    for (int i = 0; i < DP; ++i)
#pragma unroll
                        for (int j = 0; j < DP; ++j) {
                            const bool in = (i < D && j < D);
                            const double sg = in ? s_Sig[i * D + j] : 0.0;
                            const double dab = in ? c_ils2[a * E + j] + c_ils2[a * E + j] : 0.0;
                            m[i][j] = sg * dab + (i == j ? 1.0 : 0.0);
                            m[i][DP + j] = sg;
                        }
                    s_rdiag[a] = 1.0 / sqrt(small_solve<DP>(m));
                } else if (first && wave == 3) {
                    for (int a = 0; a < D; ++a) {
                        const double* tp = p.tile_part + ((size_t)c * D + a) * p.ntiles;
                        double v = 0.0;
                        for (int k = lane; k < p.ntiles; k += 64) v += tp[k];
                        v = wave_sum(v);
                        if (lane == 0) s_rdiag[4 + a] = v;
                    }
                }
            }
#if defined(GPMPC_PROF_ON)
            if (threadIdx.x == 0 && blockIdx.x == 0) { long long now_ = __builtin_readcyclecounter(); prof_acc[7] += now_ - prof_last; }
            if (blockIdx.x == 0 && threadIdx.x == 64) prof_x[0] += __builtin_readcyclecounter() - prof_p1;
#endif
            if (tid == NT - 1) {
                *s_counter = 0;
                int no = 0;
                for (int gq = 0; gq < Gc; ++gq)
                    if (s_pa[q0 + gq] != s_pb[q0 + gq]) s_off[no++] = gq;
                *s_noff = no;
#if defined(GPMPC_PROF_ON)
                if (blockIdx.x == 0) prof_x[1] += __builtin_readcyclecounter() - prof_p1;
#endif
            }
            __syncthreads();
            GPMPC_TRACE(2);

            const int n_off = *s_noff;
            [[maybe_unused]] bool cl_list_pending = false;
            [[maybe_unused]] int cl_ns = 0, cl_cls = 3, cl_code0 = 0;
            if (wave == NW - 1) {
                const int wtri = (s_tri[p.RC] + 63) >> 6;
                const int R = Gc + nmean;
                int ns = 0, cls = 3, code0 = 0;
                [[maybe_unused]] unsigned long long mymask = 0;
                if (lane < Gc) {
                    const int Kr = s_K[lane];
                    const bool sep = (Kr & 64) != 0;
                    if (sep) {
                        const int Ks = Kr & 63;
                        const int two = (DX == 3) ? 2 * sep3_bands(Ks <= 3 ? 3 : Ks) : 2 * ((s_mcum[Ks] + 7) >> 3);
                        ns = two < wpp ? two : wpp;
                    } else {
                        ns = (s_pa[q0 + lane] == s_pb[q0 + lane]) ? wtri : wpp;
                    }
                    cls = sep ? 1 : 0;
                    code0 = lane * wpp;
                    s_nslot[lane] = ns;
                    if constexpr (CL) {
                        if (sep) mymask = (s_sepown[lane] == member) ? (ns >= 64 ? ~0ull : (1ull << ns) - 1ull) : 0ull;
                        else mymask = s_mymask[lane];
                    }
                } else if (lane < R) {
                    ns = 1; cls = 2; code0 = 0xffff - (lane - Gc);
                    if constexpr (CL) mymask = (s_meanown[lane - Gc] == member) ? 1ull : 0ull;
                }
                auto build_list = [&] {
                    int start = 0, total_items = 0;
                    for (int m = 0; m < R; ++m) {
                        const int nsm = __builtin_amdgcn_readlane(ns, m);
                        const int clm = __builtin_amdgcn_readlane(cls, m);
                        start += (clm < cls || (clm == cls && m < lane)) ? nsm : 0;
                        total_items += nsm;
                    }
                    for (int k = 0; k < ns; ++k) s_items[start + k] = (unsigned short)(cls == 2 ? code0 : code0 + k);
                    if (lane == 0) *s_nitems = total_items;
                    return total_items;
                };
                if constexpr (!CL) {
                    (void)build_list();
                } else if (wpp > 64) {
                    const int total_items = build_list();
                    wave_lds_sync();
                    int cnt = 0;
                    for (int base = 0; base < total_items; base += 64) {
                        const int k = base + lane;
                        const int code = s_items[k < total_items ? k : 0];
                        const bool mine = k < total_items && item_owner(code) == member;
                        const unsigned long long mask = __ballot(mine);
                        if (mine) s_mine[1 + cnt + __popcll(mask & ((1ull << lane) - 1ull))] = (unsigned short)code;
                        cnt += __popcll(mask);
                    }
                    if (lane == 0) s_mine[0] = (unsigned short)cnt;
                } else {
                    const int mycnt = __popcll(mymask);
                    int pre = 0, tot = 0, total_items = 0;
                    for (int m = 0; m < R; ++m) {
                        const int cm = __builtin_amdgcn_readlane(mycnt, m);
                        const int clm = __builtin_amdgcn_readlane(cls, m);
                        pre += (clm < cls || (clm == cls && m < lane)) ? cm : 0;
                        tot += cm;
                        total_items += __builtin_amdgcn_readlane(ns, m);
                    }
                    unsigned long long mk = mymask;
                    for (int i = 0; mk != 0; ++i) {
                        const int k = __builtin_ctzll(mk);
                        mk &= mk - 1ull;
                        s_mine[1 + pre + i] = (unsigned short)(cls == 2 ? code0 : code0 + k);
                    }
                    if (lane == 0) { s_mine[0] = (unsigned short)tot; *s_nitems = total_items; }
                    cl_list_pending = true;
                    cl_ns = ns; cl_cls = cls; cl_code0 = code0;
                }
            }
            const int p2_threads = (NW >= 8) ? NT - 64 : NT;
            int p2_items = (nmean + Gc + n_off) * N;
            [[maybe_unused]] bool cl_nu_first = false;
            if (CL && (NW < 8 || wave != NW - 1)) {
                const int nall = nmean + Gc + n_off;
                bool need = false;
                int code = lane;
                if (lane < nmean) need = s_meanown[lane] == member;
                else if (lane < nmean + Gc) need = pair_needed(lane - nmean);
                else if (lane < nall) need = pair_needed(s_off[lane - nmean - Gc]);
                const unsigned long long mask0 = __ballot(need);
                if (lane == nall) { need = s_meanown[0] != member && mask0 == 0; code = 255; }
                const unsigned long long mask = __ballot(need);
                if (need) s_needw[wave * 64 + __popcll(mask & ((1ull << lane) - 1ull))] = (unsigned char)code;
                p2_items = __popcll(mask) * N;
                cl_nu_first = s_meanown[0] != member && mask0 != 0;
                wave_lds_sync();
            }
            for (int it = tid; it < p2_items && tid < p2_threads; it += p2_threads) {
                int prob = p.magic_pt ? (int)__umulhi((unsigned)it, p.magic_pt) : it;
                const int pt = it - prob * N;
                double nu[DP];
#pragma unroll
                for (int d = 0; d < DP; ++d) nu[d] = (d < D) ? (Xs[d * N + pt] - s_m[d]) : 0.0;
                if constexpr (CL) {
                    if (cl_nu_first && prob == 0) {
#pragma unroll
                        for (int d = 0; d < DP; ++d)
                            if (d < D) a_nu[d * N + pt] = nu[d];
                    }
                    prob = s_needw[wave * 64 + prob];
                    if (prob == 255) {
#pragma unroll
                        for (int d = 0; d < DP; ++d)
                            if (d < D) a_nu[d * N + pt] = nu[d];
                        continue;
                    }
                }
                if (prob < nmean) {
                    const int a = prob;
                    const double* Ai = s_aug + a * (D * LD) + D;
                    double q = 0.0;
#pragma unroll
                    for (int i = 0; i < DP; ++i) {
                        if (i < D) {
                            double r = 0.0;
#pragma unroll
                            for (int j = 0; j < DP; ++j)
                                if (j < D) r = fma(Ai[i * LD + j], nu[j], r);
                            q = fma(nu[i], r, q);
                        }
                    }
                    for (int e = D; e < E; ++e) {
                        const double v = Xs[e * N + pt] - s_m[e];
                        q = fma(v * v, c_ils2[a * E + e], q);
                    }
                    a_lb[a * N + pt] = fast_exp(-0.5 * q, c_exptab) * p.beta[a * N + pt];
                    if (a == 0) {
#pragma unroll
                        for (int d = 0; d < DP; ++d)
                            if (d < D) a_nu[d * N + pt] = nu[d];
                    }
                } else {
                    const bool rowside = prob < nmean + Gc;
                    const int gq = rowside ? prob - nmean : s_off[prob - nmean - Gc];
                    const int a = s_pa[q0 + gq], b = s_pb[q0 + gq];
                    const int c = rowside ? a : b;
                    const int Kw = s_K[gq];
                    const int K = Kw & 63;
                    const int sl = CL ? (Kw >> 8) - 1 : gq;
                    const double* Z = s_aug + (D + gq) * (D * LD) + D;
                    double u[DP], g[DP];
// ... 151 lines not shown
                            } else {
                                wt = a_kb[sl3 * N + pt];
#pragma unroll
                                for (int d = 0; d < DP; ++d) x[d] = (d < D) ? a_nu[d * N + pt] * c_ils2[b * E + d] : 0.0;
                            }
#pragma unroll
                            for (int m = 0; m < 8; ++m) {
                                double t = wt;
#pragma unroll
                                for (int d = 0; d < (DP < 4 ? DP : 4); ++d) {
                                    const int ne = (packed[m] >> (8 * d)) & 255;
                                    for (int e = 0; e < ne; ++e) t *= x[d];
                                }
                                acc[m] += t;
                            }
                        }
                        const double tot = wave_reduce8(acc);
                        const int mm = lane >> 2;
                        if ((lane & 3) == 0 && lane < 32 && al0 + mm < C) s_mom[(gq * 2 + side) * rnd2(CM) + al0 + mm] = tot;
                    }
                    continue;
                }
                const int flat = slot * 64 + lane;
                bool valid;
                int r, jc;
                int nrows_tab = -1;
                if (diag && use_lmap) {
                    const int packed = s_lmap[flat];
                    valid = packed >= 0;
                    r = valid ? (packed & 255) : 0;
                    jc = valid ? (packed >> 8) : 0;
                    nrows_tab = __builtin_amdgcn_readfirstlane(s_lrows[slot]);
                } else if (diag) {
                    valid = flat < s_tri[p.RC];
                    int lo = 0, hi = p.RC;
                    while (hi - lo > 1) {
                        const int mid = (lo + hi) >> 1;
                        if (s_tri[mid] <= flat) lo = mid; else hi = mid;
                    }
                    r = valid ? lo : 0;
                    const int first = C2 ? (r * p.CH) / 2 : r * p.CH;
                    jc = valid ? first + (flat - s_tri[r]) : 0;
                } else {
                    valid = flat < p.RC * NC;
                    r = valid ? (p.magic_N ? (int)__umulhi((unsigned)flat, p.magic_N) : flat) : 0;
                    jc = valid ? flat - r * NC : 0;
                }
                const int j = C2 ? 2 * jc : jc;
                const bool valid1 = C2 && (j + 1 < N);
                const int jl = valid1 ? j + 1 : j;
                const int i0 = r * p.CH;
                int i1 = i0 + p.CH;
                if (i1 > N) i1 = N;
                if (diag && i1 > jl + 1) i1 = jl + 1;
                int nrows = nrows_tab;
                if (nrows_tab < 0) {
                    const int len = (valid && i1 > i0) ? (i1 - i0) : 0;
                    nrows = (wave_max_i32(len) + 3) & ~3;
                }
                double acc = 0.0;
                if (nrows > 0) {
                    double w[DP];
#pragma unroll
                    for (int d = 0; d < DP; ++d) w[d] = (d < D) ? a_nu[d * N + j] * c_ils2[b * E + d] : 0.0;
                    const int sle = CL ? (Kraw >> 8) - 1 : gq;
                    const double kbj = a_kb[sle * N + j];
                    const double* rec = a_rows + ((size_t)sle * NR + i0) * RS;
                    [[maybe_unused]] const double* Tp = p.Tm + ((size_t)a * (N + kTPad) + i0) * N + j;
                    if constexpr (C2) {
                        const TRows trows = make_t_rows(p.Tm, D, N, a, i0, j);
                        double w1[DP];
                        const double m1 = valid1 ? 1.0 : 0.0;
#pragma unroll
                        for (int d = 0; d < DP; ++d) w1[d] = (d < D) ? a_nu[d * N + jl] * (c_ils2[b * E + d] * m1) : 0.0;
                        const double kb1 = a_kb[sle * N + jl] * m1;
                        double acc0, acc1;
                        if (K == 0) {
                            item_exp2<DP>(rec, nrows, w, w1, kbj, kb1, diag, trows, c_exptab, acc0, acc1);
                            acc = acc0 * (diag ? 2.0 : p.beta[b * N + j]) + (valid1 ? acc1 * (diag ? 2.0 : p.beta[b * N + j + 1]) : 0.0);
                        } else {
                            constexpr int TU = DP >= 4 ? 4 : 2;
                            if (K <= 2) item_taylor2<DP, 2, TU>(rec, nrows, w, w1, diag, trows, acc0, acc1);
                            else if (K == 3) item_taylor2<DP, 3, TU>(rec, nrows, w, w1, diag, trows, acc0, acc1);
                            else if (K == 4) item_taylor2<DP, 4, TU>(rec, nrows, w, w1, diag, trows, acc0, acc1);
                            else if (K == 5) item_taylor2<DP, 5, TU>(rec, nrows, w, w1, diag, trows, acc0, acc1);
                            else if (K == 6) item_taylor2<DP, 6, TU>(rec, nrows, w, w1, diag, trows, acc0, acc1);
                            else if (K == 7) item_taylor2<DP, 7, TU>(rec, nrows, w, w1, diag, trows, acc0, acc1);
                            else if (K == 8) item_taylor2<DP, 8, TU>(rec, nrows, w, w1, diag, trows, acc0, acc1);
                            else if (K <= 10) item_taylor2<DP, 10, TU>(rec, nrows, w, w1, diag, trows, acc0, acc1);
                            else if (K <= 12) item_taylor2<DP, 12, TU>(rec, nrows, w, w1, diag, trows, acc0, acc1);
                            else item_taylor2<DP, 14, TU>(rec, nrows, w, w1, diag, trows, acc0, acc1);
                            acc = fma(acc0, kbj, acc1 * kb1) * (diag ? 2.0 : 1.0);
                        }
                    } else if (K == 0) {
                        acc = item_exp<DP, REC>(rec, nrows, w, kbj, diag, Tp, N, c_exptab);
                        acc *= diag ? 2.0 : p.beta[b * N + j];
                    } else {
                        if (K <= 2) acc = item_taylor<DP, 2, REC>(rec, nrows, w, diag, Tp, N);
                        else if (K == 3) acc = item_taylor<DP, 3, REC>(rec, nrows, w, diag, Tp, N);
                        else if (K == 4) acc = item_taylor<DP, 4, REC>(rec, nrows, w, diag, Tp, N);
                        else if (K == 5) acc = item_taylor<DP, 5, REC>(rec, nrows, w, diag, Tp, N);
                        else if (K == 6) acc = item_taylor<DP, 6, REC>(rec, nrows, w, diag, Tp, N);
                        else if (K == 7) acc = item_taylor<DP, 7, REC>(rec, nrows, w, diag, Tp, N);
                        else if (K == 8) acc = item_taylor<DP, 8, REC>(rec, nrows, w, diag, Tp, N);
                        else if (K <= 10) acc = item_taylor<DP, 10, REC>(rec, nrows, w, diag, Tp, N);
                        else if (K <= 12) acc = item_taylor<DP, 12, REC>(rec, nrows, w, diag, Tp, N);
                        else acc = item_taylor<DP, 14, REC>(rec, nrows, w, diag, Tp, N);
                        acc *= diag ? 2.0 * kbj : kbj;
                    }
                    acc = valid ? acc : 0.0;
                }
                acc = wave_sum(acc);
                if (lane == 0) {
                    s_part[wi] = acc;
                    if constexpr (CL) publish(wi, acc);
                }
            }
#if defined(GPMPC_PROF_ON) && defined(GPMPC_PROF_BARRIER)
            if constexpr (CL) __syncthreads();
#endif
            GPMPC_TRACE(8);
            if constexpr (CL) {
                const bool own_sep = __ballot(lane < Gc && (s_K[lane < Gc ? lane : 0] & 64) && s_sepown[lane < Gc ? lane : 0] == member) != 0;
                __syncthreads();
                if (own_sep) {
                    for (int gq = wave; gq < Gc; gq += NW) {
                        const int Kraw = s_K[gq];
                        if (!(Kraw & 64) || s_sepown[gq] != member) continue;
                        const int C = s_mcum[Kraw & 63];
                        const double* Gm = s_mom + (gq * 2) * rnd2(CM);
                        const double* Wm = Gm + rnd2(CM);
                        double v = 0.0;
                        for (int al = lane; al < C; al += 64) v = fma(Gm[al] * Wm[al], c_monow[al], v);
                        v = wave_sum(v);
                        if (lane == 0) publish(x_sep + gq, v);
                    }
                }
                const int npair = total - nmean;
                for (int k = tid; k < npair + nmean * (D + 1); k += NT) {
                    int vi = -1;
                    double* dst = nullptr;
                    if (k < npair) {
                        const int code = s_items[k];
                        const int gq = p.magic_wpp ? (int)__umulhi((unsigned)code, p.magic_wpp) : code;
                        if (!(s_K[gq] & 64)) { vi = code; dst = s_part + code; }
                        else if (code == gq * wpp) { vi = x_sep + gq; dst = s_sepv + gq; }
                    } else {
                        vi = x_mean + (k - npair); dst = s_s1 + (k - npair);
                    }
                    if (vi >= 0) *dst = acquire(vi);
                }
            }
#if defined(GPMPC_PROF_ON)
            if (blockIdx.x == 0 && (threadIdx.x & 63) == 0) prof_x[2] += __builtin_readcyclecounter() - prof_p3;
#endif
            __syncthreads();
            GPMPC_TRACE(4);

            for (int gq = wave; gq < Gc; gq += NW) {
                const int Kraw = s_K[gq];
                double v = 0.0;
                if ((Kraw & 64) && CL) {
                    v = s_sepv[gq];
                } else {
                    if (Kraw & 64) {
                        const int C = s_mcum[Kraw & 63];
                        const double* Gm = s_mom + (gq * 2) * rnd2(CM);
                        const double* Wm = Gm + rnd2(CM);
                        for (int al = lane; al < C; al += 64) v = fma(Gm[al] * Wm[al], c_monow[al], v);
                    } else {
                        const int ns = s_nslot[gq];
                        for (int k = lane; k < ns; k += 64) v += s_part[gq * wpp + k];
                    }
                    v = wave_sum(v);
                }
                if constexpr (TILED) {
                    const int a = s_pa[q0 + gq], b = s_pb[q0 + gq];
                    if (lane == 0) s_Sp[a * D - (a * (a - 1)) / 2 + (b - a)] = v * s_rdet[gq];
                } else {
                    if (lane == 0) s_Sp[q0 + gq] = v * s_rdet[gq];
                }
            }
            if constexpr (TILED) {
                if (first && tid < D) s_Sp[tid * D - (tid * (tid - 1)) / 2] = 2.0 * s_rdiag[4 + tid] * s_rdiag[tid];
            }
            if (first) {
                if (tid < D) s_M[tid] = s_cc[tid] * s_s1[tid * (D + 1)];
                for (int idx = tid; idx < D * D; idx += NT) {
                    const int k = idx / D, a = idx - k * D;
                    const double* Ai = s_aug + a * (D * LD) + D;
                    double s = 0.0;
                    for (int j = 0; j < D; ++j) s = fma(Ai[k * LD + j], s_s1[a * (D + 1) + 1 + j], s);
                    s_Vs[idx] = s_cc[a] * s;
                }
            }
            __syncthreads();
            GPMPC_TRACE(5);
        }

        for (int idx = tid; idx < D * D; idx += NT) {
            const int i = idx / D, j = idx - i * D;
            const int a = i < j ? i : j, b = i < j ? j : i;
            const int q = a * D - (a * (a - 1)) / 2 + (b - a);
            const double S = s_Sp[q] - s_M[i] * s_M[j] + (i == j ? c_var[i] : 0.0);
            double cij = 0.0, cji = 0.0;
            for (int k = 0; k < D; ++k) {
                cij = fma(s_Sig[i * D + k], s_Vs[k * D + j], cij);
                cji = fma(s_Sig[j * D + k], s_Vs[k * D + i], cji);
            }
            const double v = S + s_Sig[idx] + (cij + cji);
            s_SigNext[idx] = v;
            if (member == 0) p.Sig_out[((size_t)c * (H + 1) + (t + 1)) * D * D + idx] = v;
        }
        for (int i = tid; i < D; i += NT) {
            const double v = s_mu[i] + s_M[i];
            s_mu[i] = v;
            if (member == 0) p.mu_out[((size_t)c * (H + 1) + (t + 1)) * D + i] = v;
        }
        cur ^= 1;
        __syncthreads();
        if constexpr (CL) {
            if (*s_fail) {
                if (member == 0) {
                    for (int i = tid; i < (H - t) * D; i += NT) p.mu_out[((size_t)c * (H + 1) + (t + 1)) * D + i] = __builtin_nan("");
                    for (int i = tid; i < (H - t) * D * D; i += NT) p.Sig_out[((size_t)c * (H + 1) + (t + 1)) * D * D + i] = __builtin_nan("");
                }
                return;
            }
        }
        GPMPC_TRACE(6);
    }
#if defined(GPMPC_PROF_ON)
    if (threadIdx.x == 0 && blockIdx.x == 0) printf("PROF wave0 small algebra cycles %lld\n", prof_acc[7]);
    if (blockIdx.x == 0 && threadIdx.x == 64) printf("PROF P1 pair problems done after %lld cycles (summed over steps)\n", prof_x[0]);
    if (blockIdx.x == 0 && threadIdx.x == NT - 1) printf("PROF P1 last thread done after %lld\n", prof_x[1]);
    if (blockIdx.x == 0 && (threadIdx.x & 63) == 0) printf("PROF P3 wave %d left the queue after %lld\n", (int)(threadIdx.x >> 6), prof_x[2]);
    if (CL && threadIdx.x == 0 && (blockIdx.x & 7) == 0)
        printf("PROF member %2d xcc %d same_xcd %d\n", member, (int)__builtin_amdgcn_s_getreg(20 | (0 << 6) | ((4 - 1) << 11)), (int)same_xcd);
    if (CL && threadIdx.x == 0 && (blockIdx.x & 7) == 0)
        printf("PROF member %2d wall (10 ns ticks): P1 %lld | P2 %lld | items(wave 0) %lld | gather+wait %lld | P4 %lld | P5 %lld\n", member,
               prof_wall[2], prof_wall[3], prof_wall[8], prof_wall[4], prof_wall[5], prof_wall[6]);
    if (threadIdx.x == 0 && blockIdx.x == 0)
        printf("PROF cycles: init %lld | P1 %lld | P2 %lld | P3 %lld (wave 0's items %lld) | P4 %lld | P5 %lld\n", prof_acc[1], prof_acc[2],
               prof_acc[3], prof_acc[4] + prof_acc[8], prof_acc[8], prof_acc[5], prof_acc[6]);
#endif
}

__device__ __forceinline__ void traj_cost_generic(int c, int lane, const double* __restrict__ mu, const double* __restrict__ Sig,
                                                          const double* __restrict__ actions, const double* __restrict__ cost,
                                                          int D, int A, int H, double kappa, int clip, int use_constraints,
                                                          double* __restrict__ cm_out, double* __restrict__ cv_out,
                                                          double* __restrict__ J_out) {
    const int DA = D + A;
    const double* target = cost;
    const double* W = cost + DA;
    const double* WT = W + DA * DA;
    const double* smin = WT + D * D;
    const double* smax = smin + D;
    double jsum = 0.0;
    for (int t = lane; t <= H; t += 64) {
        const bool terminal = (t == H);
        const int n = terminal ? D : DA;
        const double* Wm = terminal ? WT : W;
        const double* m = mu + ((size_t)c * (H + 1) + t) * D;
        const double* S = Sig + ((size_t)c * (H + 1) + t) * D * D;
        const double* a = actions + ((size_t)c * H + (terminal ? 0 : t)) * A;
        auto err = [&](int i) { return (i < D ? m[i] : a[i - D]) - target[i]; };
        double cm = 0.0, cv = 0.0;
        for (int i = 0; i < D; ++i)
            for (int j = 0; j < D; ++j) cm = fma(S[i * D + j], Wm[j * n + i], cm);
        for (int i = 0; i < n; ++i) {
            const double ei = err(i);
            for (int j = 0; j < n; ++j) cm = fma(ei * Wm[i * n + j], err(j), cm);
        }
        for (int i = 0; i < D; ++i)
            for (int j = 0; j < D; ++j) {
                double tij = 0.0, tji = 0.0;
                for (int k = 0; k < D; ++k) {
                    tij = fma(Wm[i * n + k], S[k * D + j], tij);
                    tji = fma(Wm[j * n + k], S[k * D + i], tji);
                }
                cv = fma(2.0 * tij, tji, cv);
                double v1 = 0.0, v2 = 0.0;
                for (int k = 0; k < n; ++k) {
                    v1 = fma(err(k), Wm[k * n + i], v1);
                    v2 = fma(Wm[j * n + k], err(k), v2);
                }
                cv = fma(4.0 * v1 * S[i * D + j], v2, cv);
            }
        if (use_constraints && !terminal) {
            for (int d = 0; d < D; ++d) {
                const double sg = S[d * D + d];
                cm += 0.5 * (1.0 + erf((smin[d] - m[d]) / (sg * 1.4142135623730951)))
                    + (1.0 - 0.5 * (1.0 + erf((smax[d] - m[d]) / (sg * 1.4142135623730951))));
            }
        }
        double ucb = -cm + kappa * sqrt(cv);
        if (clip) ucb = fmin(ucb, 0.0);
        jsum -= ucb;
        if (cm_out) cm_out[(size_t)c * (H + 1) + t] = cm;
        if (cv_out) cv_out[(size_t)c * (H + 1) + t] = cv;
    }
    jsum = wave_xor_sum(jsum);
    if (lane == 0 && J_out) J_out[c] = jsum / (double)(H + 1);
}

template <int D, int N>
__device__ __forceinline__ void stage_cost_terms(const double* S, const double* e, const double* Wm, double& cm_out, double& cv_out) {
    double cm = 0.0, cv = 0.0;
#pragma unroll
    for (int i = 0; i < D; ++i)
#pragma unroll
        for (int j = 0; j < D; ++j) cm = fma(S[i * D + j], Wm[j * N + i], cm);
#pragma unroll
    for (int i = 0; i < N; ++i) {
        const double ei = e[i];
#pragma unroll
        for (int j = 0; j < N; ++j) cm = fma(ei * Wm[i * N + j], e[j], cm);
    }
#pragma unroll
    for (int i = 0; i < D; ++i)
#pragma unroll
        for (int j = 0; j < D; ++j) {
            double tij = 0.0, tji = 0.0;
#pragma unroll
            for (int k = 0; k < D; ++k) {
                tij = fma(Wm[i * N + k], S[k * D + j], tij);
                tji = fma(Wm[j * N + k], S[k * D + i], tji);
            }
            cv = fma(2.0 * tij, tji, cv);
            double v1 = 0.0, v2 = 0.0;
#pragma unroll
            for (int k = 0; k < N; ++k) {
                v1 = fma(e[k], Wm[k * N + i], v1);
                v2 = fma(Wm[j * N + k], e[k], v2);
            }
            cv = fma(4.0 * v1 * S[i * D + j], v2, cv);
        }
    cm_out = cm;
    cv_out = cv;
}

template <int D, int A>
__device__ __forceinline__ void traj_cost_fixed(int c, int lane, const double* __restrict__ mu, const double* __restrict__ Sig,
                                                        const double* __restrict__ actions, const double* __restrict__ cost,
                                                        int H, double kappa, int clip, int use_constraints,
                                                        double* __restrict__ cm_out, double* __restrict__ cv_out,
                                                        double* __restrict__ J_out) {
    constexpr int DA = D + A;
    double target[DA], W[DA * DA], WT[D * D], smin[D], smax[D];
#pragma unroll
    for (int i = 0; i < DA; ++i) target[i] = cost[i];
#pragma unroll
    for (int i = 0; i < DA * DA; ++i) W[i] = cost[DA + i];
#pragma unroll
    for (int i = 0; i < D * D; ++i) WT[i] = cost[DA + DA * DA + i];
#pragma unroll
    for (int d = 0; d < D; ++d) {
        smin[d] = cost[DA + DA * DA + D * D + d];
        smax[d] = cost[DA + DA * DA + D * D + D + d];
    }
    double jsum = 0.0;
    for (int t = lane; t <= H; t += 64) {
        const bool terminal = (t == H);
        const double* mp = mu + ((size_t)c * (H + 1) + t) * D;
        const double* Sp = Sig + ((size_t)c * (H + 1) + t) * D * D;
        const double* ap = actions + ((size_t)c * H + (terminal ? 0 : t)) * A;
        double S[D * D], m[D], e[DA];
#pragma unroll
        for (int i = 0; i < D * D; ++i) S[i] = Sp[i];
#pragma unroll
        for (int i = 0; i < D; ++i) m[i] = mp[i];
#pragma unroll
        for (int i = 0; i < A; ++i) e[D + i] = (terminal ? 0.0 : ap[i]) - target[D + i];
#pragma unroll
        for (int i = 0; i < D; ++i) e[i] = m[i] - target[i];
        double cm, cv;
        if (terminal) stage_cost_terms<D, D>(S, e, WT, cm, cv);
        else stage_cost_terms<D, DA>(S, e, W, cm, cv);
        if (use_constraints && !terminal) {
#pragma unroll
            for (int d = 0; d < D; ++d) {
                const double sg = S[d * D + d];
                cm += 0.5 * (1.0 + erf((smin[d] - m[d]) / (sg * 1.4142135623730951)))
                    + (1.0 - 0.5 * (1.0 + erf((smax[d] - m[d]) / (sg * 1.4142135623730951))));
            }
        }
        double ucb = -cm + kappa * sqrt(cv);
        if (clip) ucb = fmin(ucb, 0.0);
// ... 29 lines not shown
```

### data-efficient-reinforcement-learning-with-probabilistic-model-predictive-control_amd/engine.py

```python
import ctypes as C

import numpy as np
import torch

from . import _lib as L


def _host(a, shape=None):
    a = np.ascontiguousarray(np.asarray(a, dtype=np.float64))
    if shape is not None and a.shape != tuple(shape):
        raise ValueError(f"expected shape {tuple(shape)}, got {a.shape}")
    return a


def _hp(a):
    return a.ctypes.data_as(C.c_void_p)


def feedback_gains_layout(shape, B, H, A, D):
    shape = tuple(int(s) for s in shape)
    if shape == (A, D):
        return False, True
    if shape == (H, A, D):
        return False, False
# ... 24 lines not shown
        return {k: flat[lo:hi].reshape(sh) for k, lo, hi, sh in self.fields}


class HipEngine:

    def __init__(self, device=None):
        if not torch.cuda.is_available():
            raise RuntimeError("HipEngine needs a ROCm GPU: the GP-MPC hot path has no CPU fallback")
        self.lib = L.lib()
        self.device = torch.device("cuda", torch.cuda.current_device() if device is None else int(device))
        h = C.c_void_p()
        rc = self.lib.gpmpc_create(C.byref(h), self.device.index)
        if rc != L.GPMPC_OK:
            raise L.GpmpcError(rc, "gpmpc_create failed")
        self._h = h
        self._ogh_plans = {}
        self.N = self.D = self.E = 0
        self._cost = None

    def close(self):
        if getattr(self, "_h", None):
            self.lib.gpmpc_destroy(self._h)
            self._h = None

    def __del__(self):
        try:
            self.close()
        except Exception:
            pass

    def _check(self, rc):
        if rc == L.GPMPC_OK:
            return
        msg = self.lib.gpmpc_last_error(self._h).decode()
        if rc == L.GPMPC_ERR_NOT_PD:
            raise L.NotPositiveDefiniteError(rc, msg)
        raise L.GpmpcError(rc, msg)

    def _dev(self, t, shape=None):
        t = torch.as_tensor(t, dtype=torch.float64).to(self.device).contiguous()
        if shape is not None and tuple(t.shape) != tuple(shape):
            raise ValueError(f"expected shape {tuple(shape)}, got {tuple(t.shape)}")
        return t

    def _stream(self):
        return C.c_void_p(torch.cuda.current_stream(self.device).cuda_stream)

    def set_option(self, name, value):
        self._check(self.lib.gpmpc_set_option(self._h, name.encode(), int(value)))

    def prepare(self, X, Y, lengthscales, outputscales, noises):
        X = self._dev(X)
        N, E = X.shape
        Y = self._dev(Y)
        D = Y.shape[1]
        ls = self._dev(lengthscales, (D, E))
        osc = self._dev(outputscales).reshape(D)
        nz = self._dev(noises).reshape(D)
        self._keep = (X, Y, ls, osc, nz)
        self._check(self.lib.gpmpc_prepare(self._h, X.data_ptr(), Y.data_ptr(), ls.data_ptr(), osc.data_ptr(),
                                           nz.data_ptr(), N, D, E, self._stream()))
        self.N, self.D, self.E = N, D, E

    def prepare_sparse(self, X, Y, Z, lengthscales, outputscales, noises, jitter_rel=1e-6):
        X = self._dev(X)
        N, E = X.shape
        Y = self._dev(Y)
        D = Y.shape[1]
        if Y.shape[0] != N:
            raise ValueError(f"expected targets of shape ({N}, D), got {tuple(Y.shape)}")
        Z = self._dev(Z)
        if Z.dim() != 2 or Z.shape[1] != E:
            raise ValueError(f"expected inducing inputs of shape (M, {E}), got {tuple(Z.shape)}")
        M = Z.shape[0]
        ls = self._dev(lengthscales, (D, E))
        osc = self._dev(outputscales).reshape(D)
        nz = self._dev(noises).reshape(D)
        self._keep = (X, Y, Z, ls, osc, nz)
        self._check(self.lib.gpmpc_prepare_sparse(self._h, X.data_ptr(), Y.data_ptr(), N, Z.data_ptr(), M, ls.data_ptr(),
                                                  osc.data_ptr(), nz.data_ptr(), float(jitter_rel), D, E, self._stream()))
        self.N, self.D, self.E = M, D, E

    def _sparse_update(self, entry, X, Y):
        X = self._dev(X)
        Y = self._dev(Y)
        if X.dim() != 2 or Y.dim() != 2 or X.shape[0] != Y.shape[0]:
            raise ValueError(f"expected inputs (k, E) and targets (k, D), got {tuple(X.shape)} and {tuple(Y.shape)}")
        k, E = X.shape
        D = Y.shape[1]
        self._check(entry(self._h, X.data_ptr(), Y.data_ptr(), int(k), int(D), int(E), self._stream()))
        return X, Y

    def sparse_append(self, X_new, Y_new):
        self._keep_append = self._sparse_update(self.lib.gpmpc_sparse_append, X_new, Y_new)

    def sparse_forget(self, X_old, Y_old):
        self._sparse_update(self.lib.gpmpc_sparse_forget, X_old, Y_old)

    def select_inducing(self, X, M, lengthscales, outputscales, jitter_rel=1e-6):
        X = self._dev(X)
        if X.dim() != 2:
            raise ValueError(f"expected inputs of shape (N, E), got {tuple(X.shape)}")
        N, E = X.shape
        ls = self._dev(lengthscales)
        if ls.dim() != 2 or ls.shape[1] != E:
            raise ValueError(f"expected lengthscales of shape (D, {E}), got {tuple(ls.shape)}")
        D = ls.shape[0]
        osc = self._dev(outputscales).reshape(-1)
        if osc.numel() != D:
            raise ValueError(f"expected {D} outputscales, got {osc.numel()}")
        M = int(M)
        idx = torch.empty(max(M, 0), dtype=torch.int32, device=self.device)
        Z = torch.empty((max(M, 0), E), dtype=torch.float64, device=self.device)
        trace = torch.empty(max(M, 0), dtype=torch.float64, device=self.device)
        self._check(self.lib.gpmpc_select_inducing(self._h, X.data_ptr(), N, M, ls.data_ptr(), osc.data_ptr(), float(jitter_rel),
                                                   D, E, idx.data_ptr(), Z.data_ptr(), trace.data_ptr(), self._stream()))
        self._keep_select = (X, ls, osc)
        return {"idx": idx, "Z": Z, "trace": trace}

    def mll(self, X, Y, lengthscales, outputscales, noises):
        X = self._dev(X)
        N, E = X.shape
        Y = self._dev(Y)
        D = Y.shape[1]
        ls = self._dev(lengthscales, (D, E))
        osc = self._dev(outputscales).reshape(D)
        nz = self._dev(noises).reshape(D)
        out = np.empty((D, E + 3), dtype=np.float64)
        self._check(self.lib.gpmpc_mll(self._h, X.data_ptr(), Y.data_ptr(), ls.data_ptr(), osc.data_ptr(), nz.data_ptr(),
                                       N, D, E, out.ctypes.data_as(C.POINTER(C.c_double)), self._stream()))
        self.N, self.D, self.E = N, D, E
        return {"loss": out[:, 0].copy(), "d_lengthscale": out[:, 1:1 + E].copy(), "d_outputscale": out[:, 1 + E].copy(),
                "d_noise": out[:, 2 + E].copy()}

    def forget(self, indices):
        idx = np.asarray(indices).reshape(-1)
        if idx.size and not np.issubdtype(idx.dtype, np.integer):
            raise TypeError("forget: indices must be integers")
        idx = np.ascontiguousarray(np.clip(idx, -1, 2 ** 31 - 1), dtype=np.int32)
        self._check(self.lib.gpmpc_forget(self._h, idx.ctypes.data_as(C.POINTER(C.c_int)), int(idx.size), self._stream()))
        self.N -= int(idx.size)

    @property
    def last_prepare_mode(self):
        return int(self.lib.gpmpc_last_prepare_mode(self._h))

    @property
    def last_rollout_path(self):
        return int(self.lib.gpmpc_last_rollout_path(self._h))

    @property
    def last_cluster(self):
        return int(self.lib.gpmpc_last_cluster(self._h))

    @property
    def last_grad_path(self):
        return int(self.lib.gpmpc_last_grad_path(self._h))

    @property
    def build_id(self):
        return self.lib.gpmpc_build_id().decode()

    def set_factors(self, X, iK, beta, lengthscales, outputscales):
        X = self._dev(X)
        N, E = X.shape
        beta = self._dev(beta)
        D = beta.shape[0]
        iK = self._dev(iK, (D, N, N))
        ls = self._dev(lengthscales, (D, E))
        osc = self._dev(outputscales).reshape(D)
        self._check(self.lib.gpmpc_set_factors(self._h, X.data_ptr(), iK.data_ptr(), beta.data_ptr(), ls.data_ptr(),
                                               osc.data_ptr(), N, D, E, self._stream()))
        torch.cuda.current_stream(self.device).synchronize()
        self.N, self.D, self.E = N, D, E

    def factors(self):
        iK = torch.empty((self.D, self.N, self.N), dtype=torch.float64, device=self.device)
        beta = torch.empty((self.D, self.N), dtype=torch.float64, device=self.device)
        self._check(self.lib.gpmpc_read_factors(self._h, iK.data_ptr(), beta.data_ptr(), self._stream()))
        return iK, beta

    def predict(self, Xq, noises=None, mean=True, var=True):
        Xq = self._dev(Xq)
        if Xq.dim() != 2:
            raise ValueError(f"expected query inputs of shape (M, E), got {tuple(Xq.shape)}")
        M, E = Xq.shape
        D = self.D
        nz = _host(noises, (D,)) if noises is not None else None
        out = {}
        if mean:
            out["mean"] = torch.empty((M, D), dtype=torch.float64, device=self.device)
        if var:
            out["var"] = torch.empty((M, D), dtype=torch.float64, device=self.device)
        self._check(self.lib.gpmpc_predict(self._h, Xq.data_ptr(), M, D, E, _hp(nz) if nz is not None else None,
                                           out["mean"].data_ptr() if mean else None,
                                           out["var"].data_ptr() if var else None, self._stream()))
        self._keep_predict = Xq
        return out

    def predict_backward(self, Xq, mean_bar=None, var_bar=None):
        Xq = self._dev(Xq)
        if Xq.dim() != 2:
            raise ValueError(f"expected query inputs of shape (M, E), got {tuple(Xq.shape)}")
        M, E = Xq.shape
        D = self.D
        mb = self._dev(mean_bar, (M, D)) if mean_bar is not None else None
        vb = self._dev(var_bar, (M, D)) if var_bar is not None else None
        out = torch.empty((M, E), dtype=torch.float64, device=self.device)
        ptr = lambda t: t.data_ptr() if t is not None else None
        self._check(self.lib.gpmpc_predict_backward(self._h, Xq.data_ptr(), M, D, E, ptr(mb), ptr(vb), out.data_ptr(),
                                                    self._stream()))
        self._keep_predict_backward = (Xq, mb, vb)
        return out

    def predict_cov(self, Xa, Xb=None, noises=None):
        Xa = self._dev(Xa)
        if Xa.dim() != 2:
            raise ValueError(f"expected query inputs of shape (Ma, E), got {tuple(Xa.shape)}")
        Ma, E = Xa.shape
        D = self.D
        Mb = Ma
        if Xb is not None:
            Xb = self._dev(Xb)
            if Xb.dim() != 2 or Xb.shape[1] != E:
                raise ValueError(f"expected query inputs of shape (Mb, {E}), got {tuple(Xb.shape)}")
            Mb = Xb.shape[0]
        nz = _host(noises, (D,)) if noises is not None else None
        out = torch.empty((D, Ma, Mb), dtype=torch.float64, device=self.device)
        if Xb is not None and Mb == 0:
            return out
        self._check(self.lib.gpmpc_predict_cov(self._h, Xa.data_ptr(), Ma, Xb.data_ptr() if Xb is not None else None, Mb, D, E,
                                               _hp(nz) if nz is not None else None, out.data_ptr(), self._stream()))
        self._keep_predict_cov = (Xa, Xb)
        return out

    def moments(self, mu, var=None, S=True, V=True):
        mu = self._dev(mu)
        if mu.dim() != 2:
            raise ValueError(f"expected input means of shape (P, E), got {tuple(mu.shape)}")
        P, E = mu.shape
        D = self.D
        vr = self._dev(var, (P, E, E)) if var is not None else None
        out = {"M": torch.empty((P, D), dtype=torch.float64, device=self.device)}
        if S:
            out["S"] = torch.empty((P, D, D), dtype=torch.float64, device=self.device)
        if V:
            out["V"] = torch.empty((P, E, D), dtype=torch.float64, device=self.device)
        self._check(self.lib.gpmpc_moments(self._h, mu.data_ptr(), vr.data_ptr() if vr is not None else None, P, D, E,
                                           out["M"].data_ptr(), out["S"].data_ptr() if S else None,
                                           out["V"].data_ptr() if V else None, self._stream()))
        self._keep_moments = (mu, vr)
        return out

    def moments_linear(self, mu, var=None, S=True, V=True):
        mu = self._dev(mu)
        if mu.dim() != 2:
            raise ValueError(f"expected input means of shape (P, E), got {tuple(mu.shape)}")
        P, E = mu.shape
        D = self.D
        vr = self._dev(var, (P, E, E)) if var is not None else None
        out = {"M": torch.empty((P, D), dtype=torch.float64, device=self.device)}
        if S:
            out["S"] = torch.empty((P, D, D), dtype=torch.float64, device=self.device)
        if V:
            out["V"] = torch.empty((P, E, D), dtype=torch.float64, device=self.device)
        self._check(self.lib.gpmpc_moments_linear(self._h, mu.data_ptr(), vr.data_ptr() if vr is not None else None, P, D, E,
                                                  out["M"].data_ptr(), out["S"].data_ptr() if S else None,
                                                  out["V"].data_ptr() if V else None, self._stream()))
        self._keep_moments_linear = (mu, vr)
        return out

    def moments_backward(self, mu, var=None, M_bar=None, S_bar=None, V_bar=None, mu_bar=True, var_bar=True):
        mu = self._dev(mu)
        if mu.dim() != 2:
            raise ValueError(f"expected input means of shape (P, E), got {tuple(mu.shape)}")
        P, E = mu.shape
        D = self.D
        vr = self._dev(var, (P, E, E)) if var is not None else None
        Mb = self._dev(M_bar, (P, D)) if M_bar is not None else None
        Sb = self._dev(S_bar, (P, D, D)) if S_bar is not None else None
        Vb = self._dev(V_bar, (P, E, D)) if V_bar is not None else None
        out = {}
        if mu_bar:
            out["mu_bar"] = torch.empty((P, E), dtype=torch.float64, device=self.device)
        if var_bar:
            out["var_bar"] = torch.empty((P, E, E), dtype=torch.float64, device=self.device)
        ptr = lambda t: t.data_ptr() if t is not None else None
        self._check(self.lib.gpmpc_moments_backward(self._h, mu.data_ptr(), ptr(vr), P, D, E, ptr(Mb), ptr(Sb), ptr(Vb),
                                                    ptr(out.get("mu_bar")), ptr(out.get("var_bar")), self._stream()))
        self._keep_moments_backward = (mu, vr, Mb, Sb, Vb)
        return out

    def moments_linear_backward(self, mu, var=None, M_bar=None, S_bar=None, V_bar=None, mu_bar=True, var_bar=True):
        mu = self._dev(mu)
        if mu.dim() != 2:
            raise ValueError(f"expected input means of shape (P, E), got {tuple(mu.shape)}")
        P, E = mu.shape
        D = self.D
        vr = self._dev(var, (P, E, E)) if var is not None else None
        Mb = self._dev(M_bar, (P, D)) if M_bar is not None else None
        Sb = self._dev(S_bar, (P, D, D)) if S_bar is not None else None
        Vb = self._dev(V_bar, (P, E, D)) if V_bar is not None else None
        out = {}
        if mu_bar:
            out["mu_bar"] = torch.empty((P, E), dtype=torch.float64, device=self.device)
        if var_bar:
# ... 368 lines not shown
```

### include/gpmpc.h

```cpp
#ifndef GPMPC_H
#define GPMPC_H
#ifdef __cplusplus
extern "C" {
#endif

typedef struct gpmpc gpmpc_t;

enum {
    GPMPC_OK = 0,
    GPMPC_ERR_ARG = -1,
    GPMPC_ERR_NOT_PD = -2,
    GPMPC_ERR_HIP = -3,
    GPMPC_ERR_LIMIT = -4
};
#define GPMPC_MAX_D 16
#define GPMPC_MAX_E 24

int gpmpc_abi_version(void);
const char* gpmpc_build_id(void);
int gpmpc_create(gpmpc_t** out, int device_id);
int gpmpc_destroy(gpmpc_t* h);
const char* gpmpc_last_error(const gpmpc_t* h);

int gpmpc_prepare(gpmpc_t* h, const double* X_dev, const double* Y_dev, const double* lengthscales_dev,
                  const double* outputscales_dev, const double* noises_dev, int N, int D, int E, void* stream);
int gpmpc_last_prepare_mode(gpmpc_t* h);

int gpmpc_forget(gpmpc_t* h, const int* idx_host, int k, void* stream);

int gpmpc_prepare_sparse(gpmpc_t* h, const double* X_dev, const double* Y_dev, int N, const double* Z_dev, int M,
                         const double* lengthscales_dev, const double* outputscales_dev, const double* noises_dev,
                         double jitter_rel, int D, int E, void* stream);

int gpmpc_sparse_append(gpmpc_t* h, const double* Xnew_dev, const double* Ynew_dev, int k, int D, int E, void* stream);

int gpmpc_sparse_forget(gpmpc_t* h, const double* Xold_dev, const double* Yold_dev, int k, int D, int E, void* stream);

int gpmpc_select_inducing(gpmpc_t* h, const double* X_dev, int N, int M, const double* lengthscales_dev,
                          const double* outputscales_dev, double jitter_rel, int D, int E,
                          int* idx_out_dev, double* Z_out_dev, double* trace_out_dev, void* stream);

int gpmpc_mll(gpmpc_t* h, const double* X_dev, const double* Y_dev, const double* lengthscales_dev,
              const double* outputscales_dev, const double* noises_dev, int N, int D, int E, double* out_host, void* stream);

int gpmpc_set_factors(gpmpc_t* h, const double* X_dev, const double* iK_dev, const double* beta_dev,
                      const double* lengthscales_dev, const double* outputscales_dev, int N, int D, int E, void* stream);
int gpmpc_get_factors(gpmpc_t* h, const double** iK_dev, const double** beta_dev);
int gpmpc_read_factors(gpmpc_t* h, double* iK_dst_dev, double* beta_dst_dev, void* stream);

int gpmpc_predict(gpmpc_t* h, const double* Xq_dev, int M, int D, int E, const double* noises_host, double* mean_out_dev,
                  double* var_out_dev, void* stream);

int gpmpc_predict_backward(gpmpc_t* h, const double* Xq_dev, int M, int D, int E, const double* mean_bar_dev,
                           const double* var_bar_dev, double* Xq_bar_out_dev, void* stream);

int gpmpc_predict_cov(gpmpc_t* h, const double* Xa_dev, int Ma, const double* Xb_dev, int Mb, int D, int E,
                      const double* noises_host, double* cov_out_dev, void* stream);

int gpmpc_moments(gpmpc_t* h, const double* mu_dev, const double* var_dev, int P, int D, int E, double* M_out_dev,
                  double* S_out_dev, double* V_out_dev, void* stream);

int gpmpc_moments_backward(gpmpc_t* h, const double* mu_dev, const double* var_dev, int P, int D, int E, const double* M_bar_dev,
                           const double* S_bar_dev, const double* V_bar_dev, double* mu_bar_out_dev, double* var_bar_out_dev,
                           void* stream);

int gpmpc_moments_linear(gpmpc_t* h, const double* mu_dev, const double* var_dev, int P, int D, int E, double* M_out_dev,
                         double* S_out_dev, double* V_out_dev, void* stream);

int gpmpc_moments_linear_backward(gpmpc_t* h, const double* mu_dev, const double* var_dev, int P, int D, int E,
                                  const double* M_bar_dev, const double* S_bar_dev, const double* V_bar_dev,
                                  double* mu_bar_out_dev, double* var_bar_out_dev, void* stream);

int gpmpc_set_option(gpmpc_t* h, const char* name, long long value);

int gpmpc_set_cost(gpmpc_t* h, const double* target_host, const double* W_host, const double* W_T_host, double kappa,
                   int clip_to_zero, const double* state_min_host, const double* state_max_host, int D, int A);

int gpmpc_rollout(gpmpc_t* h, const double* actions_dev, const double* mu0_host, const double* S0_host, int B, int H, int A,
                  int include_time, double time0, double* mu_out_dev, double* Sig_out_dev, double* cost_mu_out_dev,
                  double* cost_var_out_dev, double* J_out_dev, void* stream);
int gpmpc_last_rollout_path(gpmpc_t* h);
int gpmpc_last_cluster(gpmpc_t* h);

int gpmpc_rollout_linear(gpmpc_t* h, const double* actions_dev, const double* mu0_host, const double* S0_host, int B, int H, int A,
                         int include_time, double time0, double* mu_out_dev, double* Sig_out_dev, double* cost_mu_out_dev,
                         double* cost_var_out_dev, double* J_out_dev, void* stream);

int gpmpc_rollout_linear_feedback(gpmpc_t* h, const double* actions_dev, const double* gains_dev, int gains_per_candidate,
                                  const double* mu0_host, const double* S0_host, int B, int H, int A, int include_time,
                                  double time0, double* mu_out_dev, double* Sig_out_dev, double* cost_mu_out_dev,
                                  double* cost_var_out_dev, double* J_out_dev, void* stream);

int gpmpc_lqr_gains(gpmpc_t* h, const double* actions_dev, const double* mu0_host, int B, int H, int A, int include_time,
                    double time0, double reg, double* gains_out_dev, double* P_out_dev, int* flags_out_dev, void* stream);

int gpmpc_rollout_grad(gpmpc_t* h, const double* actions_dev, const double* mu0_host, const double* S0_host, int B, int H, int A,
                       int include_time, double time0, double* J_out_dev, double* grad_out_dev, double* mu_out_dev,
                       double* Sig_out_dev, double* cost_mu_out_dev, double* cost_var_out_dev, void* stream);
int gpmpc_last_grad_path(gpmpc_t* h);

int gpmpc_rollout_backward(gpmpc_t* h, const double* actions_dev, const double* mu0_host, const double* S0_host, int B, int H, int A,
                           int include_time, double time0, const double* mu_bar_dev, const double* Sig_bar_dev,
                           const double* cost_mu_bar_dev, const double* cost_var_bar_dev, const double* J_bar_dev,
                           double* actions_bar_out_dev, double* mu0_bar_out_dev, double* S0_bar_out_dev, void* stream);

int gpmpc_rollout_linear_backward(gpmpc_t* h, const double* actions_dev, const double* mu0_host, const double* S0_host, int B,
                                  int H, int A, int include_time, double time0, const double* mu_bar_dev,
                                  const double* Sig_bar_dev, const double* cost_mu_bar_dev, const double* cost_var_bar_dev,
                                  const double* J_bar_dev, double* actions_bar_out_dev, double* mu0_bar_out_dev,
                                  double* S0_bar_out_dev, void* stream);

int gpmpc_rollout_linear_feedback_backward(gpmpc_t* h, const double* actions_dev, const double* gains_dev, int gains_per_candidate,
                                           const double* mu0_host, const double* S0_host, int B, int H, int A, int include_time,
                                           double time0, const double* mu_bar_dev, const double* Sig_bar_dev,
                                           const double* cost_mu_bar_dev, const double* cost_var_bar_dev, const double* J_bar_dev,
                                           double* actions_bar_out_dev, double* gains_bar_out_dev, double* mu0_bar_out_dev,
                                           double* S0_bar_out_dev, void* stream);

int gpmpc_objective_grad_host(gpmpc_t* h, const double* actions_host, const double* mu0_host, const double* S0_host,
                              int H, int A, int include_time, double time0, const double** result_host, void* stream);

int gpmpc_argmin(gpmpc_t* h, const double* J_dev, int B, long long first_global_index, double* best_J_host,
                 long long* best_idx_host, void* stream);
int gpmpc_argmin_async(gpmpc_t* h, const double* J_dev, int B, long long first_global_index, const double* actions_dev, int HA,
                       double* out_dev, void* stream);
int gpmpc_argmin_export(gpmpc_t* h, const double* J_dev, int B, long long first_global_index, const double* actions_dev, int HA,
                        double* out_dev, double* out_host, void* stream);

int gpmpc_cem_search(gpmpc_t* h, const double* mu0_host, const double* S0_host, int B, int H, int A, int include_time, double time0,
                     int iterations, int n_elite, unsigned long long seed, const double* first_candidate_host, int mapper,
                     const double* max_change_host, const double* action_prev_host, const double* noise_dev, double* best_out_dev,
                     void* stream);
int gpmpc_cem_local(gpmpc_t* h, const double* mu0_host, const double* S0_host, int B_total, int first, int B_local, int H, int A,
                    int include_time, double time0, int iteration, int n_elite, unsigned long long seed,
                    const double* first_candidate_host, int mapper, const double* max_change_host, const double* action_prev_host,
                    const double* noise_dev, const double* state_dev, double* elites_out_dev, void* stream);
int gpmpc_cem_merge(gpmpc_t* h, const double* elites_dev, int lists, int n_elite, int n, int iteration, double* state_dev,
                    void* stream);

int gpmpc_rollout_timed(gpmpc_t* h, const double* actions_dev, const double* mu0_host, const double* S0_host, int B, int H, int A,
                        int include_time, double time0, double* J_out_dev, int reps, float* ms_host, void* stream);

#ifdef __cplusplus
}
#endif
#endif
```

Before: 663,900.

## Software-pipeline rollout pair-group tail into next trip and merge mean/pair solves

Restructures the per-step rollout loop into a flat trip loop over (t, pair group). The reduction and covariance-update tail of the previous trip is deferred into the next trip, run by wave 0, and the mean and pair small solves are merged into one lane-parallel pass for DP<=4. This is meant to remove block-wide barriers and shorten the serial chain between timesteps. It also raises launch-bounds min waves for DP=6 and adds a diagnostic pair-group counter. The cost is more complex control flow, with the risk of subtle ordering bugs around the cur buffer flip and step_done.

```diff
diff --git a/data-efficient-reinforcement-learning-with-probabilistic-model-predictive-control_amd/_lib.py b/data-efficient-reinforcement-learning-with-probabilistic-model-predictive-control_amd/_lib.py
--- a/data-efficient-reinforcement-learning-with-probabilistic-model-predictive-control_amd/_lib.py
+++ b/data-efficient-reinforcement-learning-with-probabilistic-model-predictive-control_amd/_lib.py
@@ -51,6 +51,7 @@
     "gpmpc_last_rollout_path": (C.c_int, [_P]),
     "gpmpc_last_grad_path": (C.c_int, [_P]),
     "gpmpc_last_cluster": (C.c_int, [_P]),
+    "gpmpc_last_pair_groups": (C.c_int, [_P]),
     "gpmpc_build_id": (C.c_char_p, []),
     "gpmpc_mll": (C.c_int, [_P, _P, _P, _P, _P, _P, _I, _I, _I, C.POINTER(_D), _P]),
     "gpmpc_set_option": (C.c_int, [_P, C.c_char_p, C.c_longlong]),
diff --git a/data-efficient-reinforcement-learning-with-probabilistic-model-predictive-control_amd/csrc/abi.hip b/data-efficient-reinforcement-learning-with-probabilistic-model-predictive-control_amd/csrc/abi.hip
--- a/data-efficient-reinforcement-learning-with-probabilistic-model-predictive-control_amd/csrc/abi.hip
+++ b/data-efficient-reinforcement-learning-with-probabilistic-model-predictive-control_amd/csrc/abi.hip
@@ -398,6 +398,7 @@
 
 int gpmpc_last_rollout_path(gpmpc_t* g) { return g ? g->h.last_rollout_path : GPMPC_ERR_ARG; }
 int gpmpc_last_cluster(gpmpc_t* g) { return g ? g->h.last_cluster : GPMPC_ERR_ARG; }
+int gpmpc_last_pair_groups(gpmpc_t* g) { return g ? g->h.last_pair_groups : GPMPC_ERR_ARG; }
 
 int gpmpc_last_grad_path(gpmpc_t* g) { return g ? g->h.last_grad_path : GPMPC_ERR_ARG; }
 
diff --git a/data-efficient-reinforcement-learning-with-probabilistic-model-predictive-control_amd/csrc/gpmpc_internal.h b/data-efficient-reinforcement-learning-with-probabilistic-model-predictive-control_amd/csrc/gpmpc_internal.h
--- a/data-efficient-reinforcement-learning-with-probabilistic-model-predictive-control_amd/csrc/gpmpc_internal.h
+++ b/data-efficient-reinforcement-learning-with-probabilistic-model-predictive-control_amd/csrc/gpmpc_internal.h
@@ -209,6 +209,7 @@
     int opt_cluster = 0;
     int opt_cl_dbg = 0;
     int last_cluster = 1;
+    int last_pair_groups = 1;
     Buf mono_w;
     int* mono_exp = nullptr;
     int mono_D = -1;
diff --git a/data-efficient-reinforcement-learning-with-probabilistic-model-predictive-control_amd/csrc/rollout.hip b/data-efficient-reinforcement-learning-with-probabilistic-model-predictive-control_amd/csrc/rollout.hip
--- a/data-efficient-reinforcement-learning-with-probabilistic-model-predictive-control_amd/csrc/rollout.hip
+++ b/data-efficient-reinforcement-learning-with-probabilistic-model-predictive-control_amd/csrc/rollout.hip
@@ -407,6 +407,10 @@
     }
     h->last_rollout_path = p.path;
     h->last_cluster = p.cluster;
+    {
+        const int Pk = tiled ? a.D * (a.D - 1) / 2 : a.D * (a.D + 1) / 2;
+        h->last_pair_groups = (p.path == 1 || p.G < 1 || Pk < 1) ? 1 : (Pk + p.G - 1) / p.G;
+    }
     return GPMPC_OK;
 }
 
diff --git a/data-efficient-reinforcement-learning-with-probabilistic-model-predictive-control_amd/csrc/rollout_kernel.h b/data-efficient-reinforcement-learning-with-probabilistic-model-predictive-control_amd/csrc/rollout_kernel.h
--- a/data-efficient-reinforcement-learning-with-probabilistic-model-predictive-control_amd/csrc/rollout_kernel.h
+++ b/data-efficient-reinforcement-learning-with-probabilistic-model-predictive-control_amd/csrc/rollout_kernel.h
@@ -611,7 +611,7 @@
 }
 
 template <int DP, bool CL>
-constexpr int rollout_min_waves() { return (DP == 2 || (DP == 3 && !CL)) ? 4 : 1; }
+constexpr int rollout_min_waves() { return (DP == 2 || (DP == 3 && !CL)) ? 4 : (DP == 6 ? 3 : 1); }
 
 template <int DP, int NT, int DX, bool C2, bool TILED = false, bool CL = false>
 __global__ __launch_bounds__(NT, (rollout_min_waves<DP, CL>())) void rollout_kernel(const RolloutArgs p) {
@@ -630,6 +630,8 @@
     const int member = CL ? (spread ? (int)blockIdx.x % CS : (int)(blockIdx.x >> 3) % CS) : 0;
     const int c = CL ? (spread ? (int)blockIdx.x / CS : (int)(blockIdx.x & 7) + 8 * ((int)(blockIdx.x >> 3) / CS)) : (int)blockIdx.x;
     if constexpr (CL) { if (c >= p.B) return; }
+    constexpr bool kMerged = !CL && DX > 0 && DP <= 4;
+    constexpr bool kTailInTrip = DX == 0 || DP > 4;
     const int D = (DX > 0) ? DX : p.D;
     const int N = p.N, A = p.A, E = p.E, H = p.H, G = p.G, CM = p.CM;
     const int P = TILED ? D * (D - 1) / 2 : D * (D + 1) / 2;
@@ -709,11 +711,13 @@
     const double* act = p.actions + (size_t)c * H * A;
 
 #if defined(GPMPC_PROF_ON)
-    long long prof_x[3] = {0, 0, 0};
+    long long prof_left = 0;
     long long prof_acc[10] = {0, 0, 0, 0, 0, 0, 0, 0, 0, 0};
     long long prof_last = __builtin_readcyclecounter();
     long long prof_wall[10] = {0, 0, 0, 0, 0, 0, 0, 0, 0, 0};
     long long prof_wlast = wall_clock64();
+    long long prof_b3 = 0, prof_chain = 0;
+    int prof_chain_n = 0;
 #endif
     if constexpr (TILED) {
         for (int i = tid; i < D; i += NT) { s_mu[i] = p.mu_out[((size_t)c * (H + 1) + p.t_begin) * D + i]; c_logvar[i] = p.logvar[i]; c_var[i] = p.var[i]; }
@@ -911,152 +915,334 @@
 
     int cur = 0;
     const int tid_outer = tid;
-    for (int t = TILED ? p.t_begin : 0; t < (TILED ? p.t_end : H); ++t) {
+    const int t_last = TILED ? p.t_end : H;
+    int t = TILED ? p.t_begin : 0, q0 = 0;
+    bool have_prev = false;
+    int pq0 = 0;
+    double* traj_mu = p.mu_out + ((size_t)c * (H + 1) + (t + 1)) * D;
+    double* traj_Sig = p.Sig_out + ((size_t)c * (H + 1) + (t + 1)) * D * D;
+    for (;;) {
         int tid_opaque = tid_outer;
         asm volatile("" : "+v"(tid_opaque));
         const int tid = tid_opaque;
         const int lane = tid & 63;
         const int wave = tid >> 6;
+        const bool more = t < t_last;
+        const bool step_done = have_prev && pq0 + G >= P;
+        const double* s_SigOld = s_Sig2 + cur * SD2;
+        if (step_done) cur ^= 1;
         const double* s_Sig = s_Sig2 + cur * SD2;
-        double* s_SigNext = s_Sig2 + (cur ^ 1) * SD2;
         if constexpr (CL) {
             x_tag = p.xch_tag0 + (unsigned)t + 1u;
             x_cur = (same_xcd ? xbuf : xbuf_uc) + (size_t)(t & 1) * 2 * p.xch_n;
         }
 
-        for (int q0 = 0; q0 < P || (TILED && q0 == 0); q0 += G) {
+        {
             const int Gc = (P - q0 < G) ? (P - q0) : G;
             const bool first = (q0 == 0);
             const int nmean = first ? D : 0;
 
-            constexpr int kPairBase = (NT >= 256) ? 64 : 0;
+            if (!kTailInTrip && have_prev) {
+                const int pGc = (P - pq0 < G) ? (P - pq0) : G;
+                const bool pfirst = (pq0 == 0);
+                for (int gq = wave; gq < pGc; gq += NW) {
+                    const int Kraw = s_K[gq];
+                    double v = 0.0;
+                    if ((Kraw & 64) && CL) {
+                        v = s_sepv[gq];
+                    } else {
+                        if (Kraw & 64) {
+                            const int C = s_mcum[Kraw & 63];
+                            const double* Gm = s_mom + (gq * 2) * rnd2(CM);
+                            const double* Wm = Gm + rnd2(CM);
+                            for (int al = lane; al < C; al += 64) v = fma(Gm[al] * Wm[al], c_monow[al], v);
+                        } else {
+                            const int ns = s_nslot[gq];
+                            for (int k = lane; k < ns; k += 64) v += s_part[gq * wpp + k];
+                        }
+                        v = wave_sum(v);
+                    }
+                    if constexpr (TILED) {
+                        const int a = s_pa[pq0 + gq], b = s_pb[pq0 + gq];
+                        if (lane == 0) s_Sp[a * D - (a * (a - 1)) / 2 + (b - a)] = v * s_rdet[gq];
+                    } else {
+                        if (lane == 0) s_Sp[pq0 + gq] = v * s_rdet[gq];
+                    }
+                }
+                if (pfirst && wave == (pGc < NW ? pGc : NW - 1)) {
+                    if constexpr (TILED) {
+                        if (lane < D) s_Sp[lane * D - (lane * (lane - 1)) / 2] = 2.0 * s_rdiag[4 + lane] * s_rdiag[lane];
+                    }
+                    if (lane < D) s_M[lane] = s_cc[lane] * s_s1[lane * (D + 1)];
+                    for (int idx = lane; idx < D * D; idx += 64) {
+                        const int k = idx / D, a = idx - k * D;
+                        const double* Ai = s_aug + a * (D * LD) + D;
+                        double s = 0.0;
+                        for (int j = 0; j < D; ++j) s = fma(Ai[k * LD + j], s_s1[a * (D + 1) + 1 + j], s);
+                        s_Vs[idx] = s_cc[a] * s;
+                    }
+                }
+                __syncthreads();
+                GPMPC_TRACE(5);
+            }
+            if (!kTailInTrip && wave == 0 && have_prev) {
+                if (step_done) {
+                    wave_lds_sync();
+                    double* s_SigNext = s_Sig2 + cur * SD2;
+                    for (int idx = lane; idx < D * D; idx += 64) {
+                        const int i = idx / D, j = idx - i * D;
+                        const int a = i < j ? i : j, b = i < j ? j : i;
+                        const int q = a * D - (a * (a - 1)) / 2 + (b - a);
+                        const double S = s_Sp[q] - s_M[i] * s_M[j] + (i == j ? c_var[i] : 0.0);
+                        double cij = 0.0, cji = 0.0;
+                        for (int k = 0; k < D; ++k) {
+                            cij = fma(s_SigOld[i * D + k], s_Vs[k * D + j], cij);
+                            cji = fma(s_SigOld[j * D + k], s_Vs[k * D + i], cji);
+                        }
+                        const double v = S + s_SigOld[idx] + (cij + cji);
+                        s_SigNext[idx] = v;
+                        if (member == 0) traj_Sig[idx] = v;
+                    }
+                    for (int i = lane; i < D; i += 64) {
+                        const double v = s_mu[i] + s_M[i];
+                        s_mu[i] = v;
+                        if (member == 0) traj_mu[i] = v;
+                    }
+                }
+                wave_lds_sync();
+                GPMPC_TRACE(6);
+            }
+            if constexpr (!kMerged) {
+                if (step_done) __syncthreads();
+            }
+            if constexpr (kMerged) {
+                if (wave == 0 && more) {
+                    if (first) {
+                        for (int i = lane; i < E; i += 64) {
+                            double v;
+                            if (i < D) v = s_mu[i];
+                            else if (i < DA) v = c_act[t * A + (i - D)];
+                            else v = p.time0 + (double)t;
+                            s_m[i] = v;
+                        }
+                    }
+                    if (lane < nmean + Gc) {
+                        const bool is_mean = lane < nmean;
+                        const int gq = lane - nmean;
+                        const int a = is_mean ? lane : s_pa[q0 + gq], b = is_mean ? lane : s_pb[q0 + gq];
+                        double* aug = s_aug + (is_mean ? a : D + gq) * (D * LD);
+                        double prodil = 1.0;
+                        double det;
+                        double cmax = 0.0;
+                        {
+                            double m[DP][2 * DP];
+                            double ur[DP], wr[DP];
+#pragma unroll
+                            for (int i = 0; i < DP; ++i) {
+                                const double il2 = (i < D) ? c_ils2[a * E + i] : 1.0;
+                                prodil *= il2;
+#pragma unroll
+                                for (int j = 0; j < DP; ++j) {
+                                    const bool in = (i < D && j < D);
+                                    const double sg = in ? s_Sig[i * D + j] : 0.0;
+                                    const double dab = in ? c_ils2[a * E + j] + c_ils2[b * E + j] : 0.0;
+                                    const double m_mean = (in ? s_Sig[i * D + j] : 0.0) + (i == j ? 1.0 / il2 : 0.0);
+                                    const double m_pair = sg * dab + (i == j ? 1.0 : 0.0);
+                                    m[i][j] = is_mean ? m_mean : m_pair;
+                                    m[i][DP + j] = is_mean ? ((in && i == j) ? 1.0 : 0.0) : sg;
+                                }
+                            }
+                            prodil = is_mean ? prodil : 1.0;
+#pragma unroll
+                            for (int i = 0; i < DP; ++i) {
+                                const double mi = (i < D) ? s_mu[i] : 0.0;
+                                const double rg = (i < D) ? fmax(fabs(c_xr[i] - mi), fabs(c_xr[E + i] - mi)) : 0.0;
+                                ur[i] = (i < D) ? rg * c_ils2[a * E + i] : 0.0;
+                                wr[i] = (i < D) ? rg * c_ils2[b * E + i] : 0.0;
+                            }
+                            det = small_solve<DP>(m);
+                            double rowc[DP];
+#pragma unroll
+                            for (int i = 0; i < DP; ++i) {
+                                double r = 0.0;
+#pragma unroll
+                                for (int j = 0; j < DP; ++j) {
+                                    if (i < D && j < D) {
+                                        aug[i * LD + D + j] = m[i][DP + j];
+                                        r = fma(fabs(m[i][DP + j]), wr[j], r);
+                                    }
+                                }
+                                rowc[i] = r * ur[i];
+                            }
+#pragma unroll
+                            for (int i = 0; i < DP; ++i) cmax += rowc[i];
+                        }
+                        const double rs = (is_mean ? c_var[a] : 1.0) / sqrt(det * prodil);
+                        if (is_mean) {
+                            s_cc[a] = rs;
+                        } else {
+                            s_rdet[gq] = rs;
+                            int K = 0;
+                            if (p.force_path != 1 && cmax <= kTaylorMaxArg[kMaxTaylor]) {
+                                K = 1;
+#pragma unroll
+                                for (int k = 1; k < kMaxTaylor; ++k) K += (cmax > kTaylorMaxArg[k]) ? 1 : 0;
+                            }
+                            if (a != b && K > 0 && K <= p.sep_kmax && (DX != 3 || K <= 6) && p.force_path == 0) {
+                                const long long C_ = s_mcum[K < 3 ? 3 : K];
+                                const long long NBk = (s_mcum[K] + 7) / 8;
+                                const long long cost_sep = (DX == 3) ? 2 * (((N + 63) / 64) * (2 * C_ + 40) + (C_ / 8 + 4) * 70)
+                                                                     : 2 * NBk * (((N + 63) / 64) * (6 + 8 * K) + 80);
+                                const long long cost_el = (long long)N * N * (D + K + 3) / 64;
+                                if (p.force_sep || cost_sep < cost_el) K |= 64;
+                            }
+                            s_K[gq] = K;
+                        }
+                    }
 #if defined(GPMPC_PROF_ON)
-            const long long prof_p1 = __builtin_readcyclecounter();
+                    if (threadIdx.x == 0 && blockIdx.x == 0) {
+                        long long now_ = __builtin_readcyclecounter();
+                        prof_acc[7] += now_ - prof_last;
+                        if (prof_b3 != 0) { prof_chain += now_ - prof_b3; ++prof_chain_n; }
+                    }
 #endif
-            if (first) {
-                for (int i = tid; i < E; i += NT) {
-                    double v;
-                    if (i < D) v = s_mu[i];
-                    else if (i < DA) v = c_act[t * A + (i - D)];
-                    else v = p.time0 + (double)t;
-                    s_m[i] = v;
-                }
-            }
-            if (tid < nmean) {
-                const int a = tid;
-                double* aug = s_aug + a * (D * LD);
-                double prodil = 1.0;
-                double detA;
-                if constexpr (DP <= 4) {
-                    double m[DP][2 * DP];
-#pragma unroll
-                    for (int i = 0; i < DP; ++i) {
-                        const double il2 = (i < D) ? c_ils2[a * E + i] : 1.0;
-                        prodil *= il2;
-#pragma unroll
-                        for (int j = 0; j < DP; ++j) {
-                            const bool in = (i < D && j < D);
-                            m[i][j] = (in ? s_Sig[i * D + j] : 0.0) + (i == j ? 1.0 / il2 : 0.0);
-                            m[i][DP + j] = (in && i == j) ? 1.0 : 0.0;
-                        }
-                    }
-                    detA = small_solve<DP>(m);
-#pragma unroll
-                    for (int i = 0; i < DP; ++i)
-#pragma unroll
-                        for (int j = 0; j < DP; ++j)
-                            if (i < D && j < D) aug[i * LD + D + j] = m[i][DP + j];
-                } else {
-                    for (int i = 0; i < D; ++i) {
-                        const double il2 = c_ils2[a * E + i];
-                        prodil *= il2;
-                        for (int j = 0; j < D; ++j) {
-                            aug[i * LD + j] = s_Sig[i * D + j] + (i == j ? 1.0 / il2 : 0.0);
-                            aug[i * LD + D + j] = (i == j ? 1.0 : 0.0);
-                        }
-                    }
-                    detA = gauss_solve(aug, D, D, LD);
-                }
-                s_cc[a] = c_var[a] / sqrt(detA * prodil);
-            } else if (tid >= kPairBase + (kPairBase ? 0 : nmean) && tid < kPairBase + (kPairBase ? 0 : nmean) + Gc) {
-                const int gq = tid - kPairBase - (kPairBase ? 0 : nmean);
-                const int a = s_pa[q0 + gq], b = s_pb[q0 + gq];
-                double* aug = s_aug + (D + gq) * (D * LD);
-                double detR;
-                double cmax = 0.0;
-                if constexpr (DP <= 4) {
-                    double m[DP][2 * DP];
-#pragma unroll
-                    for (int i = 0; i < DP; ++i)
-#pragma unroll
-                        for (int j = 0; j < DP; ++j) {
-                            const bool in = (i < D && j < D);
-                            const double sg = in ? s_Sig[i * D + j] : 0.0;
-                            const double dab = in ? c_ils2[a * E + j] + c_ils2[b * E + j] : 0.0;
-                            m[i][j] = sg * dab + (i == j ? 1.0 : 0.0);
-                            m[i][DP + j] = sg;
-                        }
-                    double ur[DP], wr[DP];
-#pragma unroll
-                    for (int i = 0; i < DP; ++i) {
-                        const double mi = (i < D) ? s_mu[i] : 0.0;
-                        const double rg = (i < D) ? fmax(fabs(c_xr[i] - mi), fabs(c_xr[E + i] - mi)) : 0.0;
-                        ur[i] = (i < D) ? rg * c_ils2[a * E + i] : 0.0;
-                        wr[i] = (i < D) ? rg * c_ils2[b * E + i] : 0.0;
-                    }
-                    detR = small_solve<DP>(m);
-                    double rowc[DP];
-#pragma unroll
-                    for (int i = 0; i < DP; ++i) {
-                        double r = 0.0;
-#pragma unroll
-                        for (int j = 0; j < DP; ++j) {
-                            if (i < D && j < D) {
-                                aug[i * LD + D + j] = m[i][DP + j];
-                                r = fma(fabs(m[i][DP + j]), wr[j], r);
+                }
+            } else if (more) {
+                constexpr int kPairBase = (NT >= 256) ? 64 : 0;
+                if (first) {
+                    for (int i = tid; i < E; i += NT) {
+                        double v;
+                        if (i < D) v = s_mu[i];
+                        else if (i < DA) v = c_act[t * A + (i - D)];
+                        else v = p.time0 + (double)t;
+                        s_m[i] = v;
+                    }
+                }
+                if (tid < nmean) {
+                    const int a = tid;
+                    double* aug = s_aug + a * (D * LD);
+                    double prodil = 1.0;
+                    double detA;
+                    if constexpr (DP <= 4) {
+                        double m[DP][2 * DP];
+#pragma unroll
+                        for (int i = 0; i < DP; ++i) {
+                            const double il2 = (i < D) ? c_ils2[a * E + i] : 1.0;
+                            prodil *= il2;
+#pragma unroll
+                            for (int j = 0; j < DP; ++j) {
+                                const bool in = (i < D && j < D);
+                                m[i][j] = (in ? s_Sig[i * D + j] : 0.0) + (i == j ? 1.0 / il2 : 0.0);
+                                m[i][DP + j] = (in && i == j) ? 1.0 : 0.0;
                             }
                         }
-                        rowc[i] = r * ur[i];
-                    }
-#pragma unroll
-                    for (int i = 0; i < DP; ++i) cmax += rowc[i];
-                } else {
-                    for (int i = 0; i < D; ++i)
-                        for (int j = 0; j < D; ++j) {
-                            const double dab = c_ils2[a * E + j] + c_ils2[b * E + j];
-                            aug[i * LD + j] = s_Sig[i * D + j] * dab + (i == j ? 1.0 : 0.0);
-                            aug[i * LD + D + j] = s_Sig[i * D + j];
+                        detA = small_solve<DP>(m);
+#pragma unroll
+                        for (int i = 0; i < DP; ++i)
+#pragma unroll
+                            for (int j = 0; j < DP; ++j)
+                                if (i < D && j < D) aug[i * LD + D + j] = m[i][DP + j];
+                    } else {
+                        for (int i = 0; i < D; ++i) {
+                            const double il2 = c_ils2[a * E + i];
+                            prodil *= il2;
+                            for (int j = 0; j < D; ++j) {
+                                aug[i * LD + j] = s_Sig[i * D + j] + (i == j ? 1.0 / il2 : 0.0);
+                                aug[i * LD + D + j] = (i == j ? 1.0 : 0.0);
+                            }
                         }
-                    detR = gauss_solve(aug, D, D, LD);
-                    const double* Z = aug + D;
-                    for (int i = 0; i < D; ++i) {
-                        const double mi = s_mu[i];
-                        const double ui = fmax(fabs(c_xr[i] - mi), fabs(c_xr[E + i] - mi)) * c_ils2[a * E + i];
-                        for (int j = 0; j < D; ++j) {
-                            const double mj = s_mu[j];
-                            const double wj = fmax(fabs(c_xr[j] - mj), fabs(c_xr[E + j] - mj)) * c_ils2[b * E + j];
-                            cmax = fma(fabs(Z[i * LD + j]) * ui, wj, cmax);
+                        detA = gauss_solve(aug, D, D, LD);
+                    }
+                    s_cc[a] = c_var[a] / sqrt(detA * prodil);
+                } else if (tid >= kPairBase + (kPairBase ? 0 : nmean) && tid < kPairBase + (kPairBase ? 0 : nmean) + Gc) {
+                    const int gq = tid - kPairBase - (kPairBase ? 0 : nmean);
+                    const int a = s_pa[q0 + gq], b = s_pb[q0 + gq];
+                    double* aug = s_aug + (D + gq) * (D * LD);
+                    double detR;
+                    double cmax = 0.0;
+                    if constexpr (DP <= 4) {
+                        double m[DP][2 * DP];
+#pragma unroll
+                        for (int i = 0; i < DP; ++i)
+#pragma unroll
+                            for (int j = 0; j < DP; ++j) {
+                                const bool in = (i < D && j < D);
+                                const double sg = in ? s_Sig[i * D + j] : 0.0;
+                                const double dab = in ? c_ils2[a * E + j] + c_ils2[b * E + j] : 0.0;
+                                m[i][j] = sg * dab + (i == j ? 1.0 : 0.0);
+                                m[i][DP + j] = sg;
+                            }
+                        double ur[DP], wr[DP];
+#pragma unroll
+                        for (int i = 0; i < DP; ++i) {
+                            const double mi = (i < D) ? s_mu[i] : 0.0;
+                            const double rg = (i < D) ? fmax(fabs(c_xr[i] - mi), fabs(c_xr[E + i] - mi)) : 0.0;
+                            ur[i] = (i < D) ? rg * c_ils2[a * E + i] : 0.0;
+                            wr[i] = (i < D) ? rg * c_ils2[b * E + i] : 0.0;
                         }
-                    }
-                }
-                s_rdet[gq] = 1.0 / sqrt(detR);
-                int K = 0;
-                if (p.force_path != 1 && cmax <= kTaylorMaxArg[kMaxTaylor]) {
-                    K = 1;
-#pragma unroll
-                    for (int k = 1; k < kMaxTaylor; ++k) K += (cmax > kTaylorMaxArg[k]) ? 1 : 0;
-                }
-                if (a != b && K > 0 && K <= p.sep_kmax && (DX != 3 || K <= 6) && p.force_path == 0) {
-                    const long long C_ = s_mcum[K < 3 ? 3 : K];
-                    const long long NBk = (s_mcum[K] + 7) / 8;
-                    const long long cost_sep = (DX == 3) ? 2 * (((N + 63) / 64) * (2 * C_ + 40) + (C_ / 8 + 4) * 70)
-                                                         : 2 * NBk * (((N + 63) / 64) * (6 + 8 * K) + 80);
-                    const long long cost_el = (long long)N * N * (D + K + 3) / 64;
-                    if (p.force_sep || cost_sep < cost_el) K |= 64;
-                }
-                if constexpr (CL) K |= (s_slot[gq] + 1) << 8;
-                s_K[gq] = K;
-            }
+                        detR = small_solve<DP>(m);
+                        double rowc[DP];
+#pragma unroll
+                        for (int i = 0; i < DP; ++i) {
+                            double r = 0.0;
+#pragma unroll
+                            for (int j = 0; j < DP; ++j) {
+                                if (i < D && j < D) {
+                                    aug[i * LD + D + j] = m[i][DP + j];
+                                    r = fma(fabs(m[i][DP + j]), wr[j], r);
+                                }
+                            }
+                            rowc[i] = r * ur[i];
+                        }
+#pragma unroll
+                        for (int i = 0; i < DP; ++i) cmax += rowc[i];
+                    } else {
+                        for (int i = 0; i < D; ++i)
+                            for (int j = 0; j < D; ++j) {
+                                const double dab = c_ils2[a * E + j] + c_ils2[b * E + j];
+                                aug[i * LD + j] = s_Sig[i * D + j] * dab + (i == j ? 1.0 : 0.0);
+                                aug[i * LD + D + j] = s_Sig[i * D + j];
+                            }
+                        detR = gauss_solve(aug, D, D, LD);
+                        const double* Z = aug + D;
+                        for (int i = 0; i < D; ++i) {
+                            const double mi = s_mu[i];
+                            const double ui = fmax(fabs(c_xr[i] - mi), fabs(c_xr[E + i] - mi)) * c_ils2[a * E + i];
+                            for (int j = 0; j < D; ++j) {
+                                const double mj = s_mu[j];
+                                const double wj = fmax(fabs(c_xr[j] - mj), fabs(c_xr[E + j] - mj)) * c_ils2[b * E + j];
+                                cmax = fma(fabs(Z[i * LD + j]) * ui, wj, cmax);
+                            }
+                        }
+                    }
+                    s_rdet[gq] = 1.0 / sqrt(detR);
+                    int K = 0;
+                    if (p.force_path != 1 && cmax <= kTaylorMaxArg[kMaxTaylor]) {
+                        K = 1;
+#pragma unroll
+                        for (int k = 1; k < kMaxTaylor; ++k) K += (cmax > kTaylorMaxArg[k]) ? 1 : 0;
+                    }
+                    if (a != b && K > 0 && K <= p.sep_kmax && (DX != 3 || K <= 6) && p.force_path == 0) {
+                        const long long C_ = s_mcum[K < 3 ? 3 : K];
+                        const long long NBk = (s_mcum[K] + 7) / 8;
+                        const long long cost_sep = (DX == 3) ? 2 * (((N + 63) / 64) * (2 * C_ + 40) + (C_ / 8 + 4) * 70)
+                                                             : 2 * NBk * (((N + 63) / 64) * (6 + 8 * K) + 80);
+                        const long long cost_el = (long long)N * N * (D + K + 3) / 64;
+                        if (p.force_sep || cost_sep < cost_el) K |= 64;
+                    }
+                    if constexpr (CL) K |= (s_slot[gq] + 1) << 8;
+                    s_K[gq] = K;
+                }
+#if defined(GPMPC_PROF_ON)
+                if (threadIdx.x == 0 && blockIdx.x == 0) { long long now_ = __builtin_readcyclecounter(); prof_acc[7] += now_ - prof_last; }
+                if (blockIdx.x == 0 && (threadIdx.x == 0 || threadIdx.x == kPairBase) && prof_b3 != 0) {
+                    prof_chain += __builtin_readcyclecounter() - prof_b3;
+                    ++prof_chain_n;
+                }
+#endif
+            }
+            if (step_done) { traj_mu += D; traj_Sig += D * D; }
+            if (!more) break;
             if constexpr (TILED) {
                 if (first && tid >= 128 && tid < 128 + D) {
                     const int a = tid - 128;
@@ -1082,19 +1268,12 @@
                     }
                 }
             }
-#if defined(GPMPC_PROF_ON)
-            if (threadIdx.x == 0 && blockIdx.x == 0) { long long now_ = __builtin_readcyclecounter(); prof_acc[7] += now_ - prof_last; }
-            if (blockIdx.x == 0 && threadIdx.x == 64) prof_x[0] += __builtin_readcyclecounter() - prof_p1;
-#endif
             if (tid == NT - 1) {
                 *s_counter = 0;
                 int no = 0;
                 for (int gq = 0; gq < Gc; ++gq)
                     if (s_pa[q0 + gq] != s_pb[q0 + gq]) s_off[no++] = gq;
                 *s_noff = no;
-#if defined(GPMPC_PROF_ON)
-                if (blockIdx.x == 0) prof_x[1] += __builtin_readcyclecounter() - prof_p1;
-#endif
             }
             __syncthreads();
             GPMPC_TRACE(2);
@@ -1552,89 +1731,99 @@
                 }
             }
 #if defined(GPMPC_PROF_ON)
-            if (blockIdx.x == 0 && (threadIdx.x & 63) == 0) prof_x[2] += __builtin_readcyclecounter() - prof_p3;
+            if (blockIdx.x == 0 && (threadIdx.x & 63) == 0) prof_left += __builtin_readcyclecounter() - prof_p3;
 #endif
             __syncthreads();
             GPMPC_TRACE(4);
-
-            for (int gq = wave; gq < Gc; gq += NW) {
-                const int Kraw = s_K[gq];
-                double v = 0.0;
-                if ((Kraw & 64) && CL) {
-                    v = s_sepv[gq];
-                } else {
-                    if (Kraw & 64) {
-                        const int C = s_mcum[Kraw & 63];
-                        const double* Gm = s_mom + (gq * 2) * rnd2(CM);
-                        const double* Wm = Gm + rnd2(CM);
-                        for (int al = lane; al < C; al += 64) v = fma(Gm[al] * Wm[al], c_monow[al], v);
+#if defined(GPMPC_PROF_ON)
+            if (blockIdx.x == 0 && (threadIdx.x & 63) == 0 && threadIdx.x <= 64) prof_b3 = __builtin_readcyclecounter();
+#endif
+            if constexpr (CL) {
+                if (*s_fail) {
+                    if (member == 0) {
+                        for (int i = tid; i < (H - t) * D; i += NT) p.mu_out[((size_t)c * (H + 1) + (t + 1)) * D + i] = __builtin_nan("");
+                        for (int i = tid; i < (H - t) * D * D; i += NT) p.Sig_out[((size_t)c * (H + 1) + (t + 1)) * D * D + i] = __builtin_nan("");
+                    }
+                    return;
+                }
+            }
+            if constexpr (kTailInTrip) {
+                for (int gq = wave; gq < Gc; gq += NW) {
+                    const int Kraw = s_K[gq];
+                    double v = 0.0;
+                    if ((Kraw & 64) && CL) {
+                        v = s_sepv[gq];
                     } else {
-                        const int ns = s_nslot[gq];
-                        for (int k = lane; k < ns; k += 64) v += s_part[gq * wpp + k];
-                    }
-                    v = wave_sum(v);
+                        if (Kraw & 64) {
+                            const int C = s_mcum[Kraw & 63];
+                            const double* Gm = s_mom + (gq * 2) * rnd2(CM);
+                            const double* Wm = Gm + rnd2(CM);
+                            for (int al = lane; al < C; al += 64) v = fma(Gm[al] * Wm[al], c_monow[al], v);
+                        } else {
+                            const int ns = s_nslot[gq];
+                            for (int k = lane; k < ns; k += 64) v += s_part[gq * wpp + k];
+                        }
+                        v = wave_sum(v);
+                    }
+                    if constexpr (TILED) {
+                        const int a = s_pa[q0 + gq], b = s_pb[q0 + gq];
+                        if (lane == 0) s_Sp[a * D - (a * (a - 1)) / 2 + (b - a)] = v * s_rdet[gq];
+                    } else {
+                        if (lane == 0) s_Sp[q0 + gq] = v * s_rdet[gq];
+                    }
                 }
                 if constexpr (TILED) {
-                    const int a = s_pa[q0 + gq], b = s_pb[q0 + gq];
-                    if (lane == 0) s_Sp[a * D - (a * (a - 1)) / 2 + (b - a)] = v * s_rdet[gq];
-                } else {
-                    if (lane == 0) s_Sp[q0 + gq] = v * s_rdet[gq];
-                }
-            }
-            if constexpr (TILED) {
-                if (first && tid < D) s_Sp[tid * D - (tid * (tid - 1)) / 2] = 2.0 * s_rdiag[4 + tid] * s_rdiag[tid];
-            }
-            if (first) {
-                if (tid < D) s_M[tid] = s_cc[tid] * s_s1[tid * (D + 1)];
-                for (int idx = tid; idx < D * D; idx += NT) {
-                    const int k = idx / D, a = idx - k * D;
-                    const double* Ai = s_aug + a * (D * LD) + D;
-                    double s = 0.0;
-                    for (int j = 0; j < D; ++j) s = fma(Ai[k * LD + j], s_s1[a * (D + 1) + 1 + j], s);
-                    s_Vs[idx] = s_cc[a] * s;
-                }
-            }
-            __syncthreads();
-            GPMPC_TRACE(5);
-        }
-
-        for (int idx = tid; idx < D * D; idx += NT) {
-            const int i = idx / D, j = idx - i * D;
-            const int a = i < j ? i : j, b = i < j ? j : i;
-            const int q = a * D - (a * (a - 1)) / 2 + (b - a);
-            const double S = s_Sp[q] - s_M[i] * s_M[j] + (i == j ? c_var[i] : 0.0);
-            double cij = 0.0, cji = 0.0;
-            for (int k = 0; k < D; ++k) {
-                cij = fma(s_Sig[i * D + k], s_Vs[k * D + j], cij);
-                cji = fma(s_Sig[j * D + k], s_Vs[k * D + i], cji);
-            }
-            const double v = S + s_Sig[idx] + (cij + cji);
-            s_SigNext[idx] = v;
-            if (member == 0) p.Sig_out[((size_t)c * (H + 1) + (t + 1)) * D * D + idx] = v;
-        }
-        for (int i = tid; i < D; i += NT) {
-            const double v = s_mu[i] + s_M[i];
-            s_mu[i] = v;
-            if (member == 0) p.mu_out[((size_t)c * (H + 1) + (t + 1)) * D + i] = v;
-        }
-        cur ^= 1;
-        __syncthreads();
-        if constexpr (CL) {
-            if (*s_fail) {
-                if (member == 0) {
-                    for (int i = tid; i < (H - t) * D; i += NT) p.mu_out[((size_t)c * (H + 1) + (t + 1)) * D + i] = __builtin_nan("");
-                    for (int i = tid; i < (H - t) * D * D; i += NT) p.Sig_out[((size_t)c * (H + 1) + (t + 1)) * D * D + i] = __builtin_nan("");
-                }
-                return;
-            }
-        }
-        GPMPC_TRACE(6);
+                    if (first && tid < D) s_Sp[tid * D - (tid * (tid - 1)) / 2] = 2.0 * s_rdiag[4 + tid] * s_rdiag[tid];
+                }
+                if (first) {
+                    if (tid < D) s_M[tid] = s_cc[tid] * s_s1[tid * (D + 1)];
+                    for (int idx = tid; idx < D * D; idx += NT) {
+                        const int k = idx / D, a = idx - k * D;
+                        const double* Ai = s_aug + a * (D * LD) + D;
+                        double s = 0.0;
+                        for (int j = 0; j < D; ++j) s = fma(Ai[k * LD + j], s_s1[a * (D + 1) + 1 + j], s);
+                        s_Vs[idx] = s_cc[a] * s;
+                    }
+                }
+                __syncthreads();
+                GPMPC_TRACE(5);
+                if (q0 + G >= P) {
+                    double* s_SigNext = s_Sig2 + (cur ^ 1) * SD2;
+                    for (int idx = tid; idx < D * D; idx += NT) {
+                        const int i = idx / D, j = idx - i * D;
+                        const int a = i < j ? i : j, b = i < j ? j : i;
+                        const int q = a * D - (a * (a - 1)) / 2 + (b - a);
+                        const double S = s_Sp[q] - s_M[i] * s_M[j] + (i == j ? c_var[i] : 0.0);
+                        double cij = 0.0, cji = 0.0;
+                        for (int k = 0; k < D; ++k) {
+                            cij = fma(s_Sig[i * D + k], s_Vs[k * D + j], cij);
+                            cji = fma(s_Sig[j * D + k], s_Vs[k * D + i], cji);
+                        }
+                        const double v = S + s_Sig[idx] + (cij + cji);
+                        s_SigNext[idx] = v;
+                        if (member == 0) p.Sig_out[((size_t)c * (H + 1) + (t + 1)) * D * D + idx] = v;
+                    }
+                    for (int i = tid; i < D; i += NT) {
+                        const double v = s_mu[i] + s_M[i];
+                        s_mu[i] = v;
+                        if (member == 0) p.mu_out[((size_t)c * (H + 1) + (t + 1)) * D + i] = v;
+                    }
+                    cur ^= 1;
+                    __syncthreads();
+                    GPMPC_TRACE(6);
+                }
+            }
+        }
+        if constexpr (!kTailInTrip) have_prev = true;
+        pq0 = q0;
+        q0 += G;
+        if (q0 >= P) { q0 = 0; ++t; }
     }
 #if defined(GPMPC_PROF_ON)
     if (threadIdx.x == 0 && blockIdx.x == 0) printf("PROF wave0 small algebra cycles %lld\n", prof_acc[7]);
-    if (blockIdx.x == 0 && threadIdx.x == 64) printf("PROF P1 pair problems done after %lld cycles (summed over steps)\n", prof_x[0]);
-    if (blockIdx.x == 0 && threadIdx.x == NT - 1) printf("PROF P1 last thread done after %lld\n", prof_x[1]);
-    if (blockIdx.x == 0 && (threadIdx.x & 63) == 0) printf("PROF P3 wave %d left the queue after %lld\n", (int)(threadIdx.x >> 6), prof_x[2]);
+    if (blockIdx.x == 0 && (threadIdx.x & 63) == 0 && prof_chain_n > 0)
+        printf("PROF chain wave %d: end of P3 -> arrival at the P1 barrier %lld cycles over %d intervals\n", (int)(threadIdx.x >> 6), prof_chain, prof_chain_n);
+    if (blockIdx.x == 0 && (threadIdx.x & 63) == 0) printf("PROF P3 wave %d left the queue after %lld\n", (int)(threadIdx.x >> 6), prof_left);
     if (CL && threadIdx.x == 0 && (blockIdx.x & 7) == 0)
         printf("PROF member %2d xcc %d same_xcd %d\n", member, (int)__builtin_amdgcn_s_getreg(20 | (0 << 6) | ((4 - 1) << 11)), (int)same_xcd);
     if (CL && threadIdx.x == 0 && (blockIdx.x & 7) == 0)
diff --git a/data-efficient-reinforcement-learning-with-probabilistic-model-predictive-control_amd/engine.py b/data-efficient-reinforcement-learning-with-probabilistic-model-predictive-control_amd/engine.py
--- a/data-efficient-reinforcement-learning-with-probabilistic-model-predictive-control_amd/engine.py
+++ b/data-efficient-reinforcement-learning-with-probabilistic-model-predictive-control_amd/engine.py
@@ -200,6 +200,10 @@
     @property
     def last_cluster(self):
         return int(self.lib.gpmpc_last_cluster(self._h))
+
+    @property
+    def last_pair_groups(self):
+        return int(self.lib.gpmpc_last_pair_groups(self._h))
 
     @property
     def last_grad_path(self):
diff --git a/include/gpmpc.h b/include/gpmpc.h
--- a/include/gpmpc.h
+++ b/include/gpmpc.h
@@ -81,6 +81,7 @@
                   double* cost_var_out_dev, double* J_out_dev, void* stream);
 int gpmpc_last_rollout_path(gpmpc_t* h);
 int gpmpc_last_cluster(gpmpc_t* h);
+int gpmpc_last_pair_groups(gpmpc_t* h);
 
 int gpmpc_rollout_linear(gpmpc_t* h, const double* actions_dev, const double* mu0_host, const double* S0_host, int B, int H, int A,
                          int include_time, double time0, double* mu_out_dev, double* Sig_out_dev, double* cost_mu_out_dev,
```

New measurement: 683,100, median of 6. 1.03x the previous value.
